# google/supersonic

Hardware: AMD Instinct MI355X
Metric: rows/sec filter->project->aggregate, 100M x 8 INT64/DOUBLE (higher is better)
Workload: dtype int64/f64; 1 GPU; Q-FPA-wide: SUM(a+b),COUNT(*),SUM(c),MIN(d),MAX(d0),SUM(d1),SUM(d2*d3) WHERE a>499 over a device-resident 100000000-row x 8-col block per GPU; rows_per_gpu=100000000, parallelism=single GPU, tile_rows=512, grid=768, lds_bytes=35568, specialized_stages=1

## Files before the change

### supersonic_amd/csrc/launch.h

```cpp
#ifndef SSGPU_LAUNCH_H_
#define SSGPU_LAUNCH_H_

#ifndef __HIPCC_RTC__
#include <hip/hip_runtime_api.h>
#include <stdint.h>
#endif
#include "vm.h"

enum SlotKind {
  SLOT_SUM_INT = 0, SLOT_SUM_DD = 1, SLOT_MIN_U64 = 2, SLOT_MAX_U64 = 3, SLOT_MIN_F64 = 4,
  SLOT_MAX_F64 = 5, SLOT_FIRST = 6, SLOT_LAST = 7, SLOT_COUNT = 8
};
enum EmitKind {
  EMIT_U64 = 0, EMIT_I64KEY = 1, EMIT_U32 = 2, EMIT_I32KEY = 3, EMIT_F64 = 4, EMIT_F32 = 5,
  EMIT_DD_F64 = 6, EMIT_DD_F32 = 7, EMIT_U8 = 8,
  EMIT_DDRES_F64 = 9,
  EMIT_CNT_U64 = 20, EMIT_CNT_U32 = 21,
  EMIT_FKEY_F64 = 100, EMIT_FKEY_F32 = 101
};
#define SSGPU_STATE_ARRAYS 8

struct EmitDesc { void* data; uint8_t* is_null; int slot; int out_kind; };

struct GroupKeyOut { void* data; uint8_t* is_null; uint32_t shift, bits, nullbit, width; };
// ... 100 lines not shown
};
hipError_t ssgpu_launch_key_domain(const PlainScatterParams& S, const unsigned int* is_signed, unsigned long long* out, int grid, hipStream_t stream);
#define SSGPU_DENSE_HEADER 64
struct DenseFoldParams {
  const void* chunks; unsigned int n_chunks, n_gaggs, any_cnt, slots;
  unsigned long long chunk_bytes;
  unsigned long long* keys; unsigned long long* acc; unsigned int* cnt;
  const unsigned int* merge_op;
  unsigned int* flags_out;
  unsigned int* clear[2]; unsigned int n_clear[2];
};
hipError_t ssgpu_launch_dense_fold(const DenseFoldParams& P, hipStream_t stream);
hipError_t ssgpu_launch_dense_headers(void* chunks, unsigned int n_chunks, unsigned long long chunk_bytes, const unsigned int* overflow4, const unsigned int* error_flag, hipStream_t stream,
                                      unsigned int forced_flags = 0);
hipError_t ssgpu_launch_hot_keys(const PlainScatterParams& S, unsigned long long n_sample, unsigned int min_count, unsigned long long* out, hipStream_t stream);
struct PscatGeom { unsigned int threads, rows, wgs_per_cu, lds, pipe; };
PscatGeom ssgpu_part_scatter_plain_geom(unsigned int n_parts, unsigned int rec_words, int threads, int rows, int wgs_per_cu);
hipError_t ssgpu_launch_part_scatter_plain(const PlainScatterParams& P, const PscatGeom& g, int grid, hipStream_t stream);
struct FoldTailColumn {
  const void* src; const unsigned char* src_nulls; void* dst; unsigned char* dst_nulls; unsigned int op, kind;
  const unsigned long long* by; const unsigned char* by_nulls;
};
hipError_t ssgpu_launch_fold_tail(const FoldTailColumn* cols_dev, unsigned int n_cols, unsigned long long n_in, unsigned long long limit, hipStream_t stream);
unsigned int ssgpu_part_scatter_plain_lds(unsigned int n_parts, unsigned int rec_words, int rows_per_thread, int threads = SSGPU_PSCAT_THREADS);
hipError_t ssgpu_part_agg_set_max_lds(int bytes);
hipError_t ssgpu_launch_group_resident(const PartAggParams& A, const PlainScatterParams& S, unsigned int lds_bytes, int grid, hipStream_t stream);

struct JoinBuildParams {
  const void* key_data[8];
  const unsigned char* key_nulls[8];
  unsigned int width[8], shift[8], bits[8];
  unsigned int n_keys;
  unsigned int capacity_mask;
  unsigned long long n_rows;
  unsigned long long* keys;
  unsigned int* rows;
  unsigned int* special;
  unsigned int* flags;
  unsigned int* counts;
  unsigned int* slot_of_row;
  unsigned int word[8];
  unsigned long long* keys_hi;
};
hipError_t ssgpu_launch_join_expand(const unsigned int* offsets, const unsigned int* run_start, const unsigned int* rows_sorted,
                                    unsigned long long n_lhs, unsigned long long n_out, unsigned int* lhs_idx, unsigned int* rhs_row, hipStream_t stream);
hipError_t ssgpu_launch_join_build(const JoinBuildParams& P, hipStream_t stream);
hipError_t ssgpu_launch_keys_ascending(const long long* keys, unsigned long long n, unsigned int* flag, hipStream_t stream);
hipError_t ssgpu_launch_fill_u32(unsigned int* p, unsigned int v, size_t n, hipStream_t stream);
struct GroupInitParams {
  unsigned long long* keys; unsigned long long n_keys;
  unsigned long long* acc; const unsigned long long* pattern; unsigned int ng; unsigned long long n_acc;
  unsigned int* cnt; unsigned long long n_cnt;
  unsigned int* z[4]; unsigned long long nz[4];
  unsigned int n_rep, pad; unsigned long long rep_stride;
};
hipError_t ssgpu_launch_group_init(const GroupInitParams& P, hipStream_t stream);

hipError_t ssgpu_launch_pipeline(const VmParams& P, int K, int grid, hipStream_t stream);
#ifndef __HIPCC_RTC__
#include <string>
void* ssgpu_rtc_specialize(int device, const VmInstr* prog, int n_instr, int K, bool math, const uint32_t* staged_width, const uint32_t* staged_lds_off,
                           int n_staged, uint32_t static_lds, std::string* why);
hipError_t ssgpu_launch_pipeline_rtc(void* handle, const VmParams& P, int grid, bool static_lds, hipStream_t stream);
void* ssgpu_rtc_specialize_part_agg(int device, const unsigned long long* desc, int n_aggs, unsigned int rec_words, unsigned int n_gaggs, bool any_cnt,
                                    unsigned int lds_bytes, std::string* why, const PlainScatterParams* source = nullptr,
                                    bool dense = false,
                                    bool prefetch = false);
hipError_t ssgpu_launch_group_resident_rtc(void* handle, const PartAggParams& A, const PlainScatterParams& S, int grid, hipStream_t stream);
hipError_t ssgpu_launch_part_agg_rtc(void* handle, const PartAggParams& P, hipStream_t stream);
void* ssgpu_rtc_specialize_pscat(int device, const PlainScatterParams& S, const PscatGeom& g, std::string* why);
hipError_t ssgpu_launch_part_scatter_plain_rtc(void* handle, const PlainScatterParams& P, const PscatGeom& g, int grid, hipStream_t stream);
void* ssgpu_rtc_function(void* handle);
void ssgpu_rtc_release(void* handle);
void ssgpu_rtc_cached_only(bool on);
void ssgpu_rtc_mode(int mode);
int ssgpu_rtc_current_mode();
bool ssgpu_rtc_pending();
void ssgpu_rtc_trim(int keep);
void ssgpu_rtc_stats(long long* modules, long long* code_bytes, long long* compilations, long long* disk_hits);
#endif
hipError_t ssgpu_pipeline_set_max_lds(int bytes);
hipError_t ssgpu_launch_finish_slots(const VmAccRec* partials, int n_slots, int n_parts, const int* slot_kind,
                                     VmAccRec* out, uint64_t* state , hipStream_t stream,
                                     const EmitDesc* descs = nullptr, int n_out = 0 );
hipError_t ssgpu_launch_slots_to_state(const VmAccRec* recs, int n_slots, const int* slot_kind, uint64_t* state,
                                       hipStream_t stream);
hipError_t ssgpu_launch_fold_state(const uint64_t* images, int n_images, uint64_t* state, int n_slots, const int* slot_kind, hipStream_t stream);
hipError_t ssgpu_launch_fold_emit(const uint64_t* images, int n_images, uint64_t* state, int n_slots, const int* slot_kind, VmAccRec* recs,
                                  const EmitDesc* descs, int n_out, hipStream_t stream);
hipError_t ssgpu_launch_state_to_slots(const uint64_t* state, int n_slots, const int* slot_kind, VmAccRec* recs,
                                       hipStream_t stream);
hipError_t ssgpu_launch_emit_scalar(const VmAccRec* recs, const EmitDesc* descs, int n_out, hipStream_t stream);
hipError_t ssgpu_launch_scan_counts(const uint32_t* in, uint32_t* out, int n, uint64_t* total, hipStream_t stream);
hipError_t ssgpu_launch_group_count(const GroupExtractParams& P, uint32_t* tile_counts, hipStream_t stream);
hipError_t ssgpu_launch_group_extract_lb(const GroupExtractParams& P, unsigned long long* status, uint64_t epoch, unsigned int* ctrl, unsigned int* error_flag, hipStream_t stream);
hipError_t ssgpu_launch_group_extract(const GroupExtractParams& P, hipStream_t stream);
hipError_t ssgpu_launch_fill_u64(uint64_t* p, uint64_t v, size_t n, hipStream_t stream);
hipError_t ssgpu_launch_fill_pattern_u64(uint64_t* p, const uint64_t* pattern, uint32_t plen, size_t n,
                                         hipStream_t stream);

hipError_t ssgpu_launch_sort_iota(uint32_t* idx, uint64_t n, hipStream_t s);
hipError_t ssgpu_launch_sort_load_keys(uint64_t* keys, const uint32_t* idx, const void* col, const uint8_t* nulls, uint32_t width,
                                       int kind, int descending, int null_pass, uint64_t n, unsigned long long* bits, hipStream_t s);
uint32_t ssgpu_sort_tiles(uint64_t n);
hipError_t ssgpu_launch_sort_hist(const uint64_t* keys, uint32_t shift, uint64_t n, uint32_t* hist, hipStream_t s);
hipError_t ssgpu_launch_sort_scatter(const uint64_t* keys_in, const uint32_t* idx_in, uint64_t* keys_out, uint32_t* idx_out,
                                     uint32_t shift, uint64_t n, const uint32_t* offsets, hipStream_t s);
hipError_t ssgpu_launch_sort_load_keys_hist(uint64_t* keys, const uint32_t* idx, const void* col, const uint8_t* nulls, uint32_t width, int kind,
                                            int descending, int null_pass, uint64_t n, unsigned long long* bits, uint32_t* hist8, uint32_t* base8, hipStream_t s,
                                            uint64_t* compact_out = nullptr);
hipError_t ssgpu_launch_sort_onesweep(const uint64_t* keys_in, const uint32_t* idx_in, uint64_t* keys_out, uint32_t* idx_out, uint32_t shift, uint64_t n,
                                      const uint32_t* digit_base, unsigned long long* status, uint32_t* ticket, uint64_t epoch, uint32_t* stuck, hipStream_t s);
hipError_t ssgpu_launch_sort_fix_ties(uint64_t* keys, uint32_t* idx, uint64_t n, uint32_t hi_shift, uint32_t* too_long, hipStream_t s);
struct SortRecField { const void* src; void* dst; unsigned int off, width; };
#define SSGPU_SORT_MAX_FIELDS 96
struct SortRecParams { void* recs; unsigned long long n; unsigned int stride, n_fields; SortRecField fields[SSGPU_SORT_MAX_FIELDS]; };
hipError_t ssgpu_launch_sort_pack(const SortRecParams& P, hipStream_t s);
hipError_t ssgpu_launch_sort_gather_rec(const SortRecParams& P, const uint32_t* idx, uint32_t idx_stride, hipStream_t s);
hipError_t ssgpu_launch_sort_fix_ties_compact(uint64_t* kc, const uint64_t* keys, uint64_t n, uint32_t* too_long, hipStream_t s);
hipError_t ssgpu_launch_sort_extract_idx(uint32_t* idx, const uint64_t* kc, uint64_t n, hipStream_t s);
struct UnpackPiece { unsigned long long src_off; void* dst; unsigned long long bytes; };
hipError_t ssgpu_launch_unpack(const char* slab, const UnpackPiece* pieces, unsigned int n_pieces, hipStream_t s);
uint64_t ssgpu_str_scan_partials(uint64_t n);
hipError_t ssgpu_launch_str_scan(uint64_t* data, uint64_t n, uint64_t* partials, hipStream_t s);
hipError_t ssgpu_launch_str_hash(const uint8_t* bytes, const uint64_t* offs, const uint8_t* nulls, uint64_t n, uint64_t* hashes, hipStream_t s);
hipError_t ssgpu_launch_str_insert(const uint8_t* bytes, const uint64_t* offs, const uint8_t* nulls, const uint64_t* hashes, uint64_t n,
                                   uint64_t* table, uint64_t cap, uint32_t* row_slot, uint32_t* error, hipStream_t s);
hipError_t ssgpu_launch_str_compact(const uint64_t* table, uint64_t cap, const uint8_t* bytes, const uint64_t* offs, uint32_t* count,
                                    uint32_t* d_slot, uint64_t* d_off, uint64_t* d_len, uint64_t* d_key, uint32_t* d_idx, hipStream_t s);
hipError_t ssgpu_launch_str_sort(uint64_t* d_key, uint32_t* d_idx, uint64_t d, uint64_t p, const uint8_t* bytes, const uint64_t* d_off,
                                 const uint64_t* d_len, hipStream_t s);
hipError_t ssgpu_launch_str_rank(const uint32_t* d_idx, const uint32_t* d_slot, const uint64_t* d_len, uint64_t d, int32_t* slot_rank,
                                 uint64_t* out_len, hipStream_t s);
hipError_t ssgpu_launch_str_codes(const uint32_t* row_slot, const uint8_t* nulls, const int32_t* slot_rank, uint64_t n, int32_t* codes, hipStream_t s);
hipError_t ssgpu_launch_str_gather(const uint8_t* bytes, const uint64_t* d_off, const uint32_t* d_idx, const uint64_t* out_off, uint64_t d,
                                   uint8_t* out, hipStream_t s);
hipError_t ssgpu_launch_str_recode(const int32_t* src, const uint8_t* nulls, const int32_t* remap, int32_t n_remap, uint64_t n, int32_t* dst,
                                   hipStream_t s);
#define STRFN_HEAP_PAD 32
hipError_t ssgpu_launch_str_fn(const uint8_t* heap, const uint64_t* offs, uint64_t n, int fn, const uint8_t* needle, uint32_t needle_len,
                               int fold, uint32_t* table, hipStream_t s);
#define STRPARSE_HARD 2
#define STRPARSE_WINDOW 64
hipError_t ssgpu_launch_str_parse(const uint8_t* heap, const uint64_t* offs, uint64_t n, int to_type, void* values, uint8_t* failed, hipStream_t s);
hipError_t ssgpu_launch_str_map_len(const uint8_t* heap, const uint64_t* offs, uint64_t n, int fn, int has_len, int64_t pos, int64_t len,
                                    uint64_t* lens, uint64_t* src, hipStream_t s);
hipError_t ssgpu_launch_str_map_write(const uint8_t* heap, const uint64_t* src, const uint64_t* dst_offs, uint64_t n, int dir, uint8_t* out, hipStream_t s);
hipError_t ssgpu_launch_str_map_compose(const int32_t* codes, uint64_t n, const int32_t* later, uint64_t n_later, uint64_t n_final, int32_t* to_final,
                                        int32_t* table, hipStream_t s);
hipError_t ssgpu_launch_str_replace_len(const uint8_t* heap, const uint64_t* offs, uint64_t n, const uint8_t* needle, uint32_t needle_len, uint32_t sub_len,
                                        uint64_t* lens, hipStream_t s);
hipError_t ssgpu_launch_str_replace_write(const uint8_t* heap, const uint64_t* offs, const uint64_t* dst_offs, uint64_t n, const uint8_t* needle, uint32_t needle_len,
                                          const uint8_t* sub, uint32_t sub_len, uint8_t* out, hipStream_t s);
hipError_t ssgpu_launch_sort_unkey(void* out, const uint64_t* keys, uint32_t width, int kind, int descending, uint64_t n, hipStream_t s);
hipError_t ssgpu_launch_sort_gather(void* out, uint8_t* out_nulls, const void* col, const uint8_t* nulls, uint32_t width,
                                    const uint32_t* idx, uint64_t n, hipStream_t s);
hipError_t ssgpu_launch_cluster_count(const void* const* data, const uint8_t* const* nulls, const uint32_t* width, uint32_t nkeys,
                                      uint64_t n, uint32_t* tile_counts, hipStream_t s);
hipError_t ssgpu_launch_cluster_flags(const void* const* data, const uint8_t* const* nulls, const uint32_t* width, uint32_t nkeys,
                                      uint64_t n, uint8_t* flag, hipStream_t s);
hipError_t ssgpu_launch_cluster_assign(const void* const* data, const uint8_t* const* nulls, const uint32_t* width, uint32_t nkeys,
                                       void* const* out_data, uint8_t* const* out_nulls, uint64_t n, const uint32_t* tile_offsets,
                                       uint32_t* seg_id, hipStream_t s);
hipError_t ssgpu_launch_gather_rowid(void* dst, const uint8_t* dst_null, const void* src, uint32_t width, int src_kind, int dst_kind, const uint64_t* rowids,
                                     uint64_t rowid_mask , int64_t row_id_base, const uint64_t* n_rows_dev, uint64_t n_rows_max, hipStream_t stream);
hipError_t ssgpu_launch_seq_sum(const void* src, const uint8_t* src_nulls, int src_kind, const uint32_t* seg_id, uint64_t n,
                                void* dst, uint8_t* dst_nulls, int dst_kind, hipStream_t s, uint64_t first = 0, uint64_t* state = nullptr, int resume = 0);
// ... 32 lines not shown
```

### supersonic_amd/csrc/pipeline_kernels.hip

```cpp
#ifndef __HIPCC_RTC__
#include <hip/hip_runtime.h>
#include <stdint.h>
#endif
#include "vm.h"
#include "launch.h"
#ifdef SSGPU_RTC_NINSTR
#include "rtc_prog.h"
#endif

typedef unsigned long long u64;
typedef long long i64;
typedef unsigned int u32;
typedef int i32;
typedef unsigned char u8;

#ifdef SSGPU_PC_PROFILE
#define PC_PROF(...) __VA_ARGS__
#else
#define PC_PROF(...)
#endif
struct LdsBase {
  __device__ __forceinline__ char* operator+(u32 off) const {
    return (char*)(__attribute__((address_space(3))) char*)off;
  }
// ... 413 lines not shown
#define KEY_APPEND_OP(OPNAME, T, UT)                                           \
  case VM_##OPNAME: { CASE_FENCE;                                              \
    const u32 shift = (u32)(I.imm & 0xFF), bits = (u32)((I.imm >> 8) & 0xFF);  \
    const u32 nullbit = (u32)((I.imm >> 16) & 0xFF);                           \
    const u64 vmask = bits >= 64 ? ~0ull : ((1ull << bits) - 1ull);            \
    _Pragma("unroll") FOR_PAIRS {                                              \
      auto kk = lds_load2<u64>(I.dst, p);                                      \
      auto vv = lds_load2<T>(I.a, p);                                          \
      u64 a0 = ((u64)(UT)vv.x) & vmask, a1 = ((u64)(UT)vv.y) & vmask;          \
      if (I.b != VM_NONE) {                                                    \
        auto z = lds_load2<u8>(I.b, p);                                        \
        if (z.x) a0 = 1ull << (nullbit - shift);                               \
        if (z.y) a1 = 1ull << (nullbit - shift);                               \
      }                                                                        \
      lds_store2<u64>(I.dst, p, kk.x | (a0 << shift), kk.y | (a1 << shift));   \
    }                                                                          \
  } break;

#define GAGG_PROLOGUE(LOADT)                                                   \
      Valid2 m = valid_pair_(p, tile_valid, I.b, VM_NONE);          \
      auto sl = lds_load2<u32>(I.c, p);                                        \
      m.x = m.x && sl.x != 0xFFFFFFFFu; m.y = m.y && sl.y != 0xFFFFFFFFu;      \
      auto vv = lds_load2<LOADT>(I.a, p);

#define GAGG_APPLY(LOADT, SL, E, ATOM)                                         \
      if ((SL) & VM_SLOT_LOCAL) {                                              \
        const u32 li = ((SL) & ~VM_SLOT_LOCAL) * P.group.local_stride + s;     \
        u64* A = reinterpret_cast<u64*>(smem + P.group.local_acc_off) + li; LOADT e = (E); ATOM; \
        if (has_cnt) atomicAdd(reinterpret_cast<u32*>(smem + P.group.local_cnt_off) + li, 1u); \
      } else {                                                                 \
        u64* A = &P.group.acc[(u64)(SL) * ng + s]; LOADT e = (E); ATOM;        \
        if (has_cnt) atomicAdd(&P.group.cnt[(u64)(SL) * ng + s], 1u);          \
      }

#define GAGG_ATOMIC(OPNAME, LOADT, ATOM)                                       \
  case VM_##OPNAME: { CASE_FENCE;                                              \
    const u32 ng = (u32)(I.imm >> 32) & 0x7FFFFFFFu, s = (u32)I.imm;           \
    const bool has_cnt = (I.imm >> 63) != 0;                                   \
    _Pragma("unroll") FOR_PAIRS {                                              \
      GAGG_PROLOGUE(LOADT)                                                     \
      if (m.x) { GAGG_APPLY(LOADT, sl.x, vv.x, ATOM) }                         \
      if (m.y) { GAGG_APPLY(LOADT, sl.y, vv.y, ATOM) }                         \
    }                                                                          \
  } break;

__device__ __noinline__ u32 lookback_rows_before(unsigned long long* status, int tile, u32 run, u64 tag, unsigned int* ctrl, unsigned int* error_flag, int lane) {
  unsigned long long* const mine = status + tile;
  if (lane == 0) __hip_atomic_store(mine, (1ull << 62) | tag | (u64)run, __ATOMIC_RELAXED, __HIP_MEMORY_SCOPE_AGENT);
  u32 excl = 0, spins = 0;
  for (int j0 = tile - 1; j0 >= 0;) {
    const int j = j0 - lane;
    u64 v = (2ull << 62) | tag;
    if (j >= 0) v = __hip_atomic_load(status + j, __ATOMIC_RELAXED, __HIP_MEMORY_SCOPE_AGENT);
    const bool ready = (v >> 62) != 0 && (v & (0x3FFFFFFFull << 32)) == tag;
    const u64 pending = __ballot(!ready), prefixes = __ballot(ready && (v >> 62) == 2);
    const u32 stop = prefixes ? (u32)__builtin_ctzll(prefixes) : 63u;
    const u64 need = stop >= 63u ? ~0ull : ((2ull << stop) - 1ull);
    if (pending & need) {
      __builtin_amdgcn_s_sleep(2);
      if (++spins > (1u << 22)) { if (lane == 0) { atomicExch(ctrl + 3, 1u); atomicExch(error_flag, 3u); } break; }
      continue;
    }
    u32 part = (u32)lane <= stop ? (u32)v : 0u;
    for (int o = 32; o > 0; o >>= 1) part += (u32)__shfl_xor((int)part, o);
    excl += part;
    if (prefixes) break;
    j0 -= 64;
  }
  if (lane == 0) __hip_atomic_store(mine, (2ull << 62) | tag | (u64)(excl + run), __ATOMIC_RELAXED, __HIP_MEMORY_SCOPE_AGENT);
  return excl;
}

__device__ __forceinline__ double vm_math1(u32 fn, double a) {
  switch (fn) {
    case VM_MATH_EXP: return exp(a);     case VM_MATH_LN: return log(a);       case VM_MATH_LOG10: return log10(a);
    case VM_MATH_LOG2: return log2(a);   case VM_MATH_SIN: return sin(a);      case VM_MATH_COS: return cos(a);
    case VM_MATH_TAN: return tan(a);     case VM_MATH_ASIN: return asin(a);    case VM_MATH_ACOS: return acos(a);
    case VM_MATH_ATAN: return atan(a);   case VM_MATH_SINH: return sinh(a);    case VM_MATH_COSH: return cosh(a);
    case VM_MATH_TANH: return tanh(a);   case VM_MATH_ASINH: return asinh(a);  case VM_MATH_ACOSH: return acosh(a);
    default: return atanh(a);
  }
}

#ifndef SSGPU_RTC_PART
template <int K, bool MATH>
__global__ __launch_bounds__(VM_WG_THREADS, VM_WAVES_PER_EU) void ssgpu_pipeline_kernel(const VmParams P) {
#ifdef SSGPU_RTC_STATIC_LDS
  __shared__ __attribute__((aligned(16))) char rtc_static_lds[SSGPU_RTC_STATIC_LDS];
  asm volatile("" ::"v"((u32)(size_t)(__attribute__((address_space(3))) char*)rtc_static_lds));
#endif
  const int t = threadIdx.x;
  const int lane = t & 63;
  const int wave = t >> 6;
  const int tile_rows = VM_TILE_UNIT * K;
  i64 vm_n_rows = P.n_rows; int vm_n_tiles = P.n_tiles;
  if (P.n_rows_dev) {
    const u64 have = *P.n_rows_dev;
    vm_n_rows = have < (u64)P.n_rows ? (i64)have : P.n_rows;
    vm_n_tiles = (int)((vm_n_rows + tile_rows - 1) / tile_rows);
  }
  const int vm_first_tile = ((P.flags & VM_FLAG_XCD_CHUNKS) && (gridDim.x & 7u) == 0u) ? (int)((blockIdx.x & 7u) * (gridDim.x >> 3) + (blockIdx.x >> 3)) : (int)blockIdx.x;
  const int n_my_tiles = vm_n_tiles > vm_first_tile ? (vm_n_tiles - vm_first_tile + (int)gridDim.x - 1) / (int)gridDim.x : 0;
  const int n_units = STAGED_COUNT(P) * K;

  for (u32 o = (u32)t * 8u; o < (u32)P.n_slots * VM_ACC_STRIDE; o += VM_COMPUTE_THREADS * 8u)
    *reinterpret_cast<u64*>(smem + P.acc_lds_off + o) = 0ull;
  typedef u64 u64xS __attribute__((ext_vector_type(VM_FAST_SLOTS)));
  typedef u32 u32xS __attribute__((ext_vector_type(VM_FAST_SLOTS)));
  u64xS F0, F1; u32xS FC;
#pragma unroll
  for (int s = 0; s < VM_FAST_SLOTS; ++s) { F0[s] = P.slot_init0[s]; F1[s] = P.slot_init1[s]; FC[s] = 0; }
  bool vm_nan_seen = false;
  for (u32 o = (u32)t * 8u; o < 2u * (u32)tile_rows; o += VM_COMPUTE_THREADS * 8u)
    *reinterpret_cast<u64*>(smem + P.const_lds_off + o) = o < (u32)tile_rows ? 0x0101010101010101ull : 0ull;

  typedef u32 u32x8 __attribute__((ext_vector_type(8)));
  typedef const __attribute__((address_space(4))) u32x8* ProgPtr;
  const ProgPtr prog0 = (ProgPtr)(P.prog);

  for (int pc = t; pc < P.n_instr; pc += VM_COMPUTE_THREADS) {
    const VmInstr J = P.prog[pc];
    const u32 w = J.imm_width;
    if (w) {
      u64 lo = J.imm;
      if (w == 4) lo = (lo & 0xFFFFFFFFull) * 0x100000001ull;
      else if (w == 1) lo = (lo & 0xFFull) * 0x0101010101010101ull;
      u64* e = reinterpret_cast<u64*>(smem + P.imm_pool_lds_off + (u32)pc * 16u);
      e[0] = lo; e[1] = lo;
    }
  }

  if (P.group.local_capacity) {
    const VmGroupTable& G = P.group;
    for (u32 e = (u32)t; e < G.local_capacity; e += VM_COMPUTE_THREADS)
      reinterpret_cast<u64*>(smem + G.local_keys_off)[e] = VM_KEY_EMPTY;
    for (u32 i = (u32)t; i < G.local_capacity * G.local_stride; i += VM_COMPUTE_THREADS) {
      reinterpret_cast<u64*>(smem + G.local_acc_off)[i] = G.acc_init[(i % G.local_stride) % G.n_gaggs];
      if (G.local_cnt_off != VM_NONE) reinterpret_cast<u32*>(smem + G.local_cnt_off)[i] = 0u;
    }
    if (t < 2) reinterpret_cast<u32*>(smem + P.scratch_lds_off + 128u)[t] = 0u;
  }
  if (P.part_n) {
    u32* h = reinterpret_cast<u32*>(smem + P.part_lds_off);
    for (u32 i = (u32)t; i < P.part_n; i += VM_COMPUTE_THREADS) h[i] = 0u;
  }
  PC_PROF(if (P.debug_pc) for (int i = t; i <= P.n_instr; i += VM_COMPUTE_THREADS) reinterpret_cast<u64*>(smem + P.debug_pc_lds_off)[i] = 0ull;)
  __syncthreads();

  u32x4 pf[VM_PF_UNITS];
#pragma unroll
  for (int u = 0; u < VM_PF_UNITS; ++u) pf[u] = u32x4{0u, 0u, 0u, 0u};
  const int n_pf = n_units < VM_PF_UNITS ? n_units : VM_PF_UNITS;
  {
    const i64 tb = (i64)vm_first_tile * tile_rows;
    if (n_my_tiles > 0 && tb + tile_rows <= vm_n_rows) {
#pragma unroll
      for (int u = 0; u < VM_PF_UNITS; ++u)
        if (u < n_pf) load_unit<K>(P, u, tb, t, pf[u]);
    }
  }

  u64 dbg_wait = 0;
  const u64 dbg_t0 = P.debug ? __builtin_amdgcn_s_memtime() : 0;
  const ProgPtr prog = prog0;
  for (int it = 0; it < n_my_tiles; ++it) {
    const int tile = vm_first_tile + it * (int)gridDim.x;
    const i64 tile_base = (i64)tile * tile_rows;
    const u32 tile_valid = (u32)((vm_n_rows - tile_base) < (i64)tile_rows ? (vm_n_rows - tile_base) : (i64)tile_rows);
    const u64 tw0 = (P.debug || P.debug_pc) ? __builtin_amdgcn_s_memtime() : 0;
    __builtin_amdgcn_s_setprio(VM_STAGE_PRIO);
    if (tile_valid == (u32)tile_rows) {
      int tc = t;
      asm volatile("" : "+v"(tc));
#pragma unroll
      for (int u = 0; u < VM_PF_UNITS; ++u)
        if (u < n_pf) commit_unit<K>(P, u, pf[u], tc);
      if (P.debug) dbg_wait += __builtin_amdgcn_s_memtime() - tw0;
      if (n_units > VM_PF_UNITS) stage_units_direct<K>(P, VM_PF_UNITS, n_units, tile_base, tile_valid, t);
    } else {
      stage_units_direct<K>(P, 0, n_units, tile_base, tile_valid, t);
    }
    {
      const i64 tb = tile_base + (i64)gridDim.x * tile_rows;
      if (it + 1 < n_my_tiles && tb + tile_rows <= vm_n_rows) {
        int tl = t;
        asm volatile("" : "+v"(tl));
#pragma unroll
        for (int u = 0; u < VM_PF_UNITS; ++u)
          if (u < n_pf) load_unit<K>(P, u, tb, tl, pf[u]);
      }
    }

    __builtin_amdgcn_s_setprio(0);
#ifdef SSGPU_RTC_NINSTR
#define VM_PC_LOOP _Pragma("unroll") for (int pc = 0; pc < SSGPU_RTC_NINSTR; ++pc)
#define VM_FETCH_NEXT(pc) u32x8{kRtcProg[pc][0], kRtcProg[pc][1], kRtcProg[pc][2], kRtcProg[pc][3], kRtcProg[pc][4], kRtcProg[pc][5], kRtcProg[pc][6], kRtcProg[pc][7]}
    (void)prog;
    u32x8 raw_next = VM_FETCH_NEXT(0);
#else
#define VM_PC_LOOP for (int pc = 0; pc < P.n_instr; ++pc)
#define VM_FETCH_NEXT(pc) prog[pc]
    u32x8 raw_next = prog[0];
#endif
    PC_PROF(u64 dbg_pc_last = 0;
    if (P.debug_pc) { dbg_pc_last = __builtin_amdgcn_s_memtime(); if (t == 0) reinterpret_cast<u64*>(smem + P.debug_pc_lds_off)[P.n_instr] += dbg_pc_last - tw0; })
#ifdef SSGPU_RTC_NINSTR
#include "rtc_steps.h"
#else
    VM_PC_LOOP {
#include "vm_body.inc"
    }
#endif
    PC_PROF(if (P.debug_pc && P.n_instr > 0 && t == 0) reinterpret_cast<u64*>(smem + P.debug_pc_lds_off)[P.n_instr - 1] += __builtin_amdgcn_s_memtime() - dbg_pc_last;)
  }

  if (vm_nan_seen && P.error_flag) atomicOr(P.error_flag, SSGPU_FLAG_NAN_IN_MINMAX);
  if (P.part_n && P.tile_counts) {
    __syncthreads();
    const u32* h = reinterpret_cast<const u32*>(smem + P.part_lds_off);
    for (u32 i = (u32)t; i < P.part_n; i += VM_COMPUTE_THREADS) P.tile_counts[(u64)i * gridDim.x + blockIdx.x] = h[i] < P.part_seg_cap ? h[i] : P.part_seg_cap;
  }
  if (P.group.local_capacity) {
    const VmGroupTable& G = P.group;
    __syncthreads();
    const u32 ng = G.n_gaggs;
    u32 occupied = 0;
    for (u32 e = (u32)t; e < G.local_capacity; e += VM_COMPUTE_THREADS) {
      const u64 key = reinterpret_cast<const u64*>(smem + G.local_keys_off)[e];
      if (key == VM_KEY_EMPTY) continue;
      ++occupied;
      const u32 gs = group_insert(G, key);
      if (gs == 0xFFFFFFFFu) continue;
      for (u32 s = 0; s < ng; ++s) {
        const u64 v = reinterpret_cast<const u64*>(smem + G.local_acc_off)[e * G.local_stride + s];
        u64* A = &G.acc[(u64)gs * ng + s];
        const u32 op = G.merge_op[s];
        if (op == VM_MERGE_ADD_U64) { if (v) atomicAdd(A, v); }
        else if (op == VM_MERGE_MIN_U64) atomicMin(A, v);
        else if (op == VM_MERGE_MAX_U64) atomicMax(A, v);
        else if (op == VM_MERGE_ADD_F64_HI) dd_atomic_add(reinterpret_cast<double*>(A), u2d(v));
        else unsafeAtomicAdd(reinterpret_cast<double*>(A), u2d(v));
        if (G.local_cnt_off != VM_NONE) {
          const u32 c = reinterpret_cast<const u32*>(smem + G.local_cnt_off)[e * G.local_stride + s];
          if (c) atomicAdd(&G.cnt[(u64)gs * ng + s], c);
        }
      }
    }
    u32* st = reinterpret_cast<u32*>(smem + P.scratch_lds_off + 128u);
    if (occupied) atomicAdd(&st[1], occupied);
    __syncthreads();
    if (t == 0) { if (st[0]) atomicAdd(&G.stats[0], st[0]); atomicMax(&G.stats[1], st[1]); }
  }

  PC_PROF(if (P.debug_pc && t == 0) for (int i = 0; i <= P.n_instr; ++i) atomicAdd(&P.debug_pc[i], reinterpret_cast<const u64*>(smem + P.debug_pc_lds_off)[i]);)
  if (P.debug && t == 0) {
    P.debug[blockIdx.x * 4 + 0] = __builtin_amdgcn_s_memtime() - dbg_t0;
    P.debug[blockIdx.x * 4 + 1] = dbg_wait;
    P.debug[blockIdx.x * 4 + 2] = (u64)n_my_tiles;
  }
#pragma unroll
  for (int s = 0; s < VM_FAST_SLOTS; ++s) {
    if (s < P.n_slots) {
      const int kind = P.slot_kind[s];
      const u64 cnt = wave_reduce_u64((u64)FC[s], [](u64 x, u64 y) { return x + y; });
      u64 v0 = 0, v1 = 0;
      switch (kind) {
        case SLOT_COUNT: v0 = cnt; break;
        case SLOT_SUM_INT: v0 = wave_reduce_u64(F0[s], [](u64 x, u64 y) { return x + y; }); break;
        case SLOT_MIN_U64: v0 = wave_reduce_u64(F0[s], [](u64 x, u64 y) { return x < y ? x : y; }); break;
        case SLOT_MAX_U64: v0 = wave_reduce_u64(F0[s], [](u64 x, u64 y) { return x > y ? x : y; }); break;
        case SLOT_MIN_F64: v0 = wave_reduce_u64(F0[s], [](u64 x, u64 y) { return u2d(y) < u2d(x) ? y : x; }); break;
        case SLOT_MAX_F64: v0 = wave_reduce_u64(F0[s], [](u64 x, u64 y) { return u2d(x) < u2d(y) ? y : x; }); break;
        case SLOT_SUM_DD: {
          DD d; d.hi = u2d(F0[s]); d.lo = u2d(F1[s]);
          d = wave_reduce_dd(d); v0 = d2u(d.hi); v1 = d2u(d.lo);
        } break;
        case SLOT_FIRST: case SLOT_LAST: {
          const bool first = kind == SLOT_FIRST;
          const u64 trow = first ? wave_reduce_u64(F1[s], [](u64 x, u64 y) { return x < y ? x : y; })
                                 : wave_reduce_u64(FC[s] ? F1[s] : 0ull, [](u64 x, u64 y) { return x > y ? x : y; });
          const u64 owner = __ballot(FC[s] != 0 && F1[s] == trow);
          const int src = owner ? __ffsll((long long)owner) - 1 : 0;
          v0 = readlane64(F0[s], src); v1 = trow;
        } break;
        default: break;
      }
      if (lane == 0) { VmAccRec* A = acc_rec(P, (u32)s, wave); A->v0 = v0; A->v1 = v1; A->cnt = cnt; A->pad = 0; }
    }
  }

  __syncthreads();
  for (int s = t; s < P.n_slots; s += VM_COMPUTE_THREADS)
    for (int w = 0; w < VM_WAVES; ++w)
      P.wg_partials[((size_t)blockIdx.x * P.n_slots + s) * VM_WAVES + w] = *acc_rec(P, (u32)s, w);
}
#endif

#ifndef __HIPCC_RTC__

__device__ __forceinline__ void combine_rec(int kind, VmAccRec& acc, const VmAccRec& r) {
  if (r.cnt == 0) return;
  switch (kind) {
    case SLOT_COUNT:
    case SLOT_SUM_INT: acc.v0 += r.v0; break;
    case SLOT_SUM_DD: {
      DD a; a.hi = u2d(acc.v0); a.lo = u2d(acc.v1);
      DD b; b.hi = u2d(r.v0); b.lo = u2d(r.v1);
      a = dd_add(a, b); acc.v0 = d2u(a.hi); acc.v1 = d2u(a.lo);
    } break;
    case SLOT_MIN_U64: acc.v0 = acc.cnt ? (r.v0 < acc.v0 ? r.v0 : acc.v0) : r.v0; break;
    case SLOT_MAX_U64: acc.v0 = acc.cnt ? (r.v0 > acc.v0 ? r.v0 : acc.v0) : r.v0; break;
    case SLOT_MIN_F64: acc.v0 = acc.cnt ? (u2d(r.v0) < u2d(acc.v0) ? r.v0 : acc.v0) : r.v0; break;
    case SLOT_MAX_F64: acc.v0 = acc.cnt ? (u2d(acc.v0) < u2d(r.v0) ? r.v0 : acc.v0) : r.v0; break;
    case SLOT_FIRST: if (!acc.cnt || r.v1 < acc.v1) { acc.v0 = r.v0; acc.v1 = r.v1; } break;
    case SLOT_LAST: if (!acc.cnt || r.v1 >= acc.v1) { acc.v0 = r.v0; acc.v1 = r.v1; } break;
  }
  acc.cnt += r.cnt;
}

__device__ __forceinline__ void slot_to_state(const VmAccRec r, int kind, int s, int n_slots, u64* __restrict__ state) {
  u64* sum_i = state; u64* cnt = state + n_slots; u64* hi = state + 2 * n_slots; u64* lo = state + 3 * n_slots;
  u64* mn = state + 4 * n_slots; u64* mx = state + 5 * n_slots;
  u64* mnf = state + 6 * n_slots; u64* mxf = state + 7 * n_slots;
  const bool fl = kind == SLOT_FIRST || kind == SLOT_LAST;
  sum_i[s] = (kind == SLOT_SUM_INT || kind == SLOT_COUNT || fl) ? r.v0 : 0;
  cnt[s] = r.cnt;
  hi[s] = kind == SLOT_SUM_DD ? r.v0 : d2u(0.0);
  lo[s] = kind == SLOT_SUM_DD ? r.v1 : d2u(0.0);
  mn[s] = (kind == SLOT_MIN_U64 && r.cnt) ? (r.v0 ^ 0x8000000000000000ull) : (kind == SLOT_FIRST && r.cnt) ? (r.v1 ^ 0x8000000000000000ull) : 0x7FFFFFFFFFFFFFFFull;
  mx[s] = (kind == SLOT_MAX_U64 && r.cnt) ? (r.v0 ^ 0x8000000000000000ull) : (kind == SLOT_LAST && r.cnt) ? (r.v1 ^ 0x8000000000000000ull) : 0x8000000000000000ull;
  mnf[s] = (kind == SLOT_MIN_F64 && r.cnt) ? r.v0 : d2u(__builtin_inf());
  mxf[s] = (kind == SLOT_MAX_F64 && r.cnt) ? r.v0 : d2u(-__builtin_inf());
}
__device__ __forceinline__ VmAccRec state_to_slot(const u64* __restrict__ state, int kind, int s, int n_slots) {
  VmAccRec r; r.v0 = 0; r.v1 = 0; r.pad = 0;
  r.cnt = state[n_slots + s];
  switch (kind) {
    case SLOT_COUNT: case SLOT_SUM_INT: r.v0 = state[s]; break;
    case SLOT_SUM_DD: {
      DD a; a.hi = u2d(state[2 * n_slots + s]); a.lo = 0.0;
      a = dd_add_d(a, u2d(state[3 * n_slots + s]));
      r.v0 = d2u(a.hi); r.v1 = d2u(a.lo);
    } break;
    case SLOT_MIN_U64: r.v0 = state[4 * n_slots + s] ^ 0x8000000000000000ull; break;
    case SLOT_MAX_U64: r.v0 = state[5 * n_slots + s] ^ 0x8000000000000000ull; break;
    case SLOT_MIN_F64: r.v0 = state[6 * n_slots + s]; break;
    case SLOT_MAX_F64: r.v0 = state[7 * n_slots + s]; break;
    case SLOT_FIRST: r.v0 = state[s]; r.v1 = state[4 * n_slots + s] ^ 0x8000000000000000ull; break;
    case SLOT_LAST: r.v0 = state[s]; r.v1 = state[5 * n_slots + s] ^ 0x8000000000000000ull; break;
    default: break;
  }
  return r;
}

__device__ __forceinline__ void emit_scalar_one(const EmitDesc d, const VmAccRec r);
__global__ __launch_bounds__(256) void ssgpu_finish_slots_kernel(const VmAccRec* __restrict__ partials, int n_slots,
                                                                 int n_parts, const int* __restrict__ slot_kind,
                                                                 VmAccRec* __restrict__ out, u64* __restrict__ state,
                                                                 const EmitDesc* __restrict__ descs, int n_out) {
  __shared__ VmAccRec tree[256];
  const int s = blockIdx.x, t = threadIdx.x;
  const int kind = slot_kind[s];
  VmAccRec acc; acc.v0 = 0; acc.v1 = 0; acc.cnt = 0; acc.pad = 0;
  if (kind == SLOT_SUM_DD) { acc.v0 = d2u(-0.0); acc.v1 = d2u(0.0); }
  for (int i = t; i < n_parts; i += 256) {
    const VmAccRec r = partials[((size_t)(i / VM_WAVES) * n_slots + s) * VM_WAVES + (i % VM_WAVES)];
    combine_rec(kind, acc, r);
  }
  tree[t] = acc;
  __syncthreads();
  for (int stride = 128; stride > 0; stride >>= 1) {
    if (t < stride) { VmAccRec a = tree[t]; combine_rec(kind, a, tree[t + stride]); tree[t] = a; }
    __syncthreads();
  }
  if (t == 0) { out[s] = tree[0]; if (state) slot_to_state(tree[0], kind, s, n_slots, state); }
  if (descs)
    for (int i = t; i < n_out; i += 256) { const EmitDesc d = descs[i]; if (d.slot == s) emit_scalar_one(d, tree[0]); }
}

__global__ void ssgpu_slots_to_state_kernel(const VmAccRec* __restrict__ recs, int n_slots,
                                            const int* __restrict__ slot_kind, u64* __restrict__ state) {
  int s = blockIdx.x * blockDim.x + threadIdx.x;
  if (s >= n_slots) return;
  slot_to_state(recs[s], slot_kind[s], s, n_slots, state);
}
__global__ void ssgpu_state_to_slots_kernel(const u64* __restrict__ state, int n_slots,
                                            const int* __restrict__ slot_kind, VmAccRec* __restrict__ recs) {
  int s = blockIdx.x * blockDim.x + threadIdx.x;
  if (s >= n_slots) return;
  recs[s] = state_to_slot(state, slot_kind[s], s, n_slots);
}


__device__ __forceinline__ void emit_value(void* dst, size_t idx, int out_kind, u64 v0, u64 v1) {
  switch (out_kind) {
    case EMIT_U64: reinterpret_cast<u64*>(dst)[idx] = v0; break;
    case EMIT_I64KEY: reinterpret_cast<i64*>(dst)[idx] = unkey_i64(v0); break;
    case EMIT_U32: reinterpret_cast<u32*>(dst)[idx] = (u32)v0; break;
    case EMIT_I32KEY: reinterpret_cast<i32*>(dst)[idx] = (i32)unkey_i64(v0); break;
    case EMIT_F64: reinterpret_cast<double*>(dst)[idx] = u2d(v0); break;
    case EMIT_F32: reinterpret_cast<float*>(dst)[idx] = (float)u2d(v0); break;
    case EMIT_DD_F64: { double hi = u2d(v0), lo = u2d(v1);
      reinterpret_cast<double*>(dst)[idx] = (lo == 0.0) ? hi : hi + lo; } break;
    case EMIT_DDRES_F64: { const double hi = u2d(v0), lo = u2d(v1), sm = hi + lo, bp = sm - hi;
      reinterpret_cast<double*>(dst)[idx] = (lo == 0.0) ? 0.0 : (hi - (sm - bp)) + (lo - bp); } break;
    case EMIT_DD_F32: { double hi = u2d(v0), lo = u2d(v1);
      reinterpret_cast<float*>(dst)[idx] = (float)((lo == 0.0) ? hi : hi + lo); } break;
    case EMIT_U8: reinterpret_cast<u8*>(dst)[idx] = (u8)(v0 != 0); break;
    default: break;
  }
}


__device__ __forceinline__ void emit_scalar_one(const EmitDesc d, const VmAccRec r) {
  if (d.out_kind == EMIT_CNT_U64 || d.out_kind == EMIT_CNT_U32)
    emit_value(d.data, 0, d.out_kind == EMIT_CNT_U64 ? EMIT_U64 : EMIT_U32, r.cnt, 0);
  else
    emit_value(d.data, 0, d.out_kind, r.v0, r.v1);
  if (d.is_null) d.is_null[0] = r.cnt == 0;
}
__global__ void ssgpu_emit_scalar_kernel(const VmAccRec* __restrict__ recs, const EmitDesc* __restrict__ descs,
                                         int n_out) {
  int i = blockIdx.x * blockDim.x + threadIdx.x;
  if (i >= n_out) return;
  const EmitDesc d = descs[i];
  emit_scalar_one(d, recs[d.slot]);
}

__global__ __launch_bounds__(1024) void ssgpu_scan_counts_kernel(const u32* __restrict__ in, u32* __restrict__ out,
                                                                  int n, u64* __restrict__ total) {
  __shared__ u64 wave_sums[16];
  __shared__ u64 carry_s;
  const int t = threadIdx.x, lane = t & 63, wave = t >> 6;
  if (t == 0) carry_s = 0;
  __syncthreads();
  for (int base = 0; base < n; base += 1024 * 8) {
    u32 v[8]; u64 sum = 0;
    int i0 = base + t * 8;
#pragma unroll
    for (int j = 0; j < 8; ++j) { v[j] = (i0 + j < n) ? in[i0 + j] : 0u; sum += v[j]; }
    u64 inc = sum;
#pragma unroll
    for (int d = 1; d < 64; d <<= 1) { u64 o = __shfl_up(inc, d); if (lane >= d) inc += o; }
    if (lane == 63) wave_sums[wave] = inc;
    __syncthreads();
    u64 wpre = 0;
    for (int w = 0; w < wave; ++w) wpre += wave_sums[w];
    u64 run = carry_s + wpre + (inc - sum);
#pragma unroll
    for (int j = 0; j < 8; ++j) { if (i0 + j < n) out[i0 + j] = (u32)run; run += v[j]; }
    __syncthreads();
    if (t == 1023) carry_s = run;
    __syncthreads();
  }
  if (t == 0) *total = carry_s;
}

__device__ __forceinline__ bool group_slot_occupied(const GroupExtractParams& P, u32 slot) {
  if (slot > P.capacity + P.extra_slots) return false;
  return P.keys[slot] != VM_KEY_EMPTY;
}

__global__ __launch_bounds__(256) void ssgpu_group_count_kernel(const GroupExtractParams P, u32* __restrict__ tile_counts) {
  __shared__ u32 wsum[4];
  const int t = threadIdx.x, lane = t & 63, wave = t >> 6;
  u32 s0 = blockIdx.x * 512u + t * 2u;
  bool o0 = group_slot_occupied(P, s0);
  bool o1 = group_slot_occupied(P, s0 + 1);
  u32 c = (u32)__popcll(__ballot(o0)) + (u32)__popcll(__ballot(o1));
  if (lane == 0) wsum[wave] = c;
  __syncthreads();
  if (t == 0) tile_counts[blockIdx.x] = wsum[0] + wsum[1] + wsum[2] + wsum[3];
}

__device__ __forceinline__ void group_extract_slot(const GroupExtractParams& P, u32 slot, u32 row);
__global__ __launch_bounds__(256) void ssgpu_group_extract_lb_kernel(const GroupExtractParams P, unsigned long long* __restrict__ status, u64 tag,
                                                                     unsigned int* __restrict__ ctrl, unsigned int* __restrict__ error_flag) {
  __shared__ u32 wsum[4];
  __shared__ u32 s_tile, s_base;
  const int t = threadIdx.x, lane = t & 63, wave = t >> 6;
  if (t == 0) s_tile = atomicAdd(ctrl + 2, 1u);
  __syncthreads();
  const u32 tile = s_tile;
  const u32 s0 = tile * 512u + (u32)t * 2u;
  const bool o0 = group_slot_occupied(P, s0), o1 = group_slot_occupied(P, s0 + 1);
  const u64 b0 = __ballot(o0), b1 = __ballot(o1);
  if (lane == 0) wsum[wave] = (u32)__popcll(b0) + (u32)__popcll(b1);
  __syncthreads();
  if (wave == 0) {
    const u32 run = wsum[0] + wsum[1] + wsum[2] + wsum[3];
    const u32 excl = lookback_rows_before(status, (int)tile, run, tag, ctrl, error_flag, lane);
    if (lane == 0) {
      s_base = excl;
      if (tile == gridDim.x - 1u) *reinterpret_cast<u64*>(ctrl) = (u64)excl + run;
    }
  }
  __syncthreads();
  u32 base = s_base;
  for (int w = 0; w < wave; ++w) base += wsum[w];
  const u64 lt = (1ull << lane) - 1ull;
  const u32 r0 = base + (u32)__popcll(b0 & lt) + (u32)__popcll(b1 & lt);
  if (o0) group_extract_slot(P, s0, r0);
  if (o1) group_extract_slot(P, s0 + 1, r0 + (o0 ? 1u : 0u));
// ... 785 lines not shown
__global__ __launch_bounds__(256) void ssgpu_gather_rowid_kernel(void* __restrict__ dst, const u8* __restrict__ dst_null, const void* __restrict__ src,
                                                                 u32 width, int src_kind, int dst_kind, const u64* __restrict__ rowids, u64 rowid_mask, i64 row_id_base,
                                                                 const u64* __restrict__ n_rows_dev, u64 n_rows_max) {
  const u64 i = (u64)blockIdx.x * 256 + threadIdx.x;
  const u64 n = n_rows_dev ? *n_rows_dev : n_rows_max;
  if (i >= n || i >= n_rows_max) return;
  const bool isnull = dst_null && dst_null[i];
  const u64 r = isnull ? 0ull : (u64)((i64)(rowids[i] & rowid_mask) - row_id_base);
  if (src_kind == dst_kind) {
    if (width == 8) reinterpret_cast<u64*>(dst)[i] = isnull ? 0ull : reinterpret_cast<const u64*>(src)[r];
    else if (width == 4) reinterpret_cast<u32*>(dst)[i] = isnull ? 0u : reinterpret_cast<const u32*>(src)[r];
    else reinterpret_cast<u8*>(dst)[i] = isnull ? (u8)0 : reinterpret_cast<const u8*>(src)[r];
    return;
  }
  i64 vi = 0; u64 vu = 0; double vf = 0.0; int fam = 0;
  if (!isnull) switch (src_kind) {
    case 0: vi = reinterpret_cast<const i32*>(src)[r]; fam = 0; break;
    case 1: vu = reinterpret_cast<const u32*>(src)[r]; fam = 1; break;
    case 2: vi = reinterpret_cast<const i64*>(src)[r]; fam = 0; break;
    case 3: vu = reinterpret_cast<const u64*>(src)[r]; fam = 1; break;
    case 4: vf = (double)reinterpret_cast<const float*>(src)[r]; fam = 2; break;
    case 5: vf = reinterpret_cast<const double*>(src)[r]; fam = 2; break;
    default: vu = reinterpret_cast<const u8*>(src)[r]; fam = 1; break;
  }
  if (dst_kind == 4 || dst_kind == 5) {
    const double d = fam == 2 ? vf : (fam == 1 ? (double)vu : (double)vi);
    if (dst_kind == 5) reinterpret_cast<double*>(dst)[i] = d;
    else reinterpret_cast<float*>(dst)[i] = fam == 2 ? (float)vf : (fam == 1 ? (float)vu : (float)vi);
    return;
  }
  u64 bits;
  if (fam == 2) {
    const double tr = trunc(vf);
    bits = (tr >= -9223372036854775808.0 && tr < 9223372036854775808.0) ? (u64)(i64)tr : 0x8000000000000000ull;
  } else bits = fam == 1 ? vu : (u64)vi;
  if (dst_kind == 2 || dst_kind == 3) reinterpret_cast<u64*>(dst)[i] = bits;
  else if (dst_kind == 0 || dst_kind == 1) reinterpret_cast<u32*>(dst)[i] = (u32)bits;
  else reinterpret_cast<u8*>(dst)[i] = (u8)bits;
}
hipError_t ssgpu_launch_gather_rowid(void* dst, const uint8_t* dst_null, const void* src, uint32_t width, int src_kind, int dst_kind, const uint64_t* rowids, uint64_t rowid_mask,
                                     int64_t row_id_base, const uint64_t* n_rows_dev, uint64_t n_rows_max, hipStream_t stream) {
  if (n_rows_max) hipLaunchKernelGGL(ssgpu_gather_rowid_kernel, dim3((unsigned)((n_rows_max + 255) / 256)), dim3(256), 0, stream,
                                     dst, dst_null, src, width, src_kind, dst_kind, (const u64*)rowids, (u64)rowid_mask, (i64)row_id_base, (const u64*)n_rows_dev, (u64)n_rows_max);
  return hipGetLastError();
}
hipError_t ssgpu_launch_fill_u32(unsigned int* p, unsigned int v, size_t n, hipStream_t stream) {
  if (n) hipLaunchKernelGGL(ssgpu_fill_u32_kernel, dim3((unsigned)std::min<size_t>((n + 255) / 256, 4096)), dim3(256), 0, stream, p, v, n);
  return hipGetLastError();
}
hipError_t ssgpu_launch_part_agg(const PartAggParams& P, unsigned int lds_bytes, hipStream_t stream) {
  if (P.rec_words <= 8) hipLaunchKernelGGL(ssgpu_part_agg_kernel<8>, dim3(P.n_parts), dim3(SSGPU_PART_THREADS), lds_bytes, stream, P);
  else if (P.rec_words <= 16) hipLaunchKernelGGL(ssgpu_part_agg_kernel<16>, dim3(P.n_parts), dim3(SSGPU_PART_THREADS), lds_bytes, stream, P);
  else if (P.rec_words <= SSGPU_PART_MAX_WORDS) hipLaunchKernelGGL(ssgpu_part_agg_kernel<SSGPU_PART_MAX_WORDS>, dim3(P.n_parts), dim3(SSGPU_PART_THREADS), lds_bytes, stream, P);
  else return hipErrorInvalidValue;
  return hipGetLastError();
}
hipError_t ssgpu_launch_group_resident(const PartAggParams& P, const PlainScatterParams& S, unsigned int lds_bytes, int grid, hipStream_t stream) {
  if (P.rec_words <= 8) hipLaunchKernelGGL(ssgpu_group_resident_kernel<8>, dim3(grid), dim3(SSGPU_PART_THREADS), lds_bytes, stream, P, S);
  else hipLaunchKernelGGL(ssgpu_group_resident_kernel<16>, dim3(grid), dim3(SSGPU_PART_THREADS), lds_bytes, stream, P, S);
  return hipGetLastError();
}
hipError_t ssgpu_part_agg_set_max_lds(int bytes) {
  hipError_t e = hipFuncSetAttribute(reinterpret_cast<const void*>(ssgpu_part_agg_kernel<8>), hipFuncAttributeMaxDynamicSharedMemorySize, bytes);
  if (e != hipSuccess) return e;
  e = hipFuncSetAttribute(reinterpret_cast<const void*>(ssgpu_group_resident_kernel<8>), hipFuncAttributeMaxDynamicSharedMemorySize, bytes);
  if (e != hipSuccess) return e;
  e = hipFuncSetAttribute(reinterpret_cast<const void*>(ssgpu_group_resident_kernel<16>), hipFuncAttributeMaxDynamicSharedMemorySize, bytes);
  if (e != hipSuccess) return e;
  e = hipFuncSetAttribute(reinterpret_cast<const void*>(ssgpu_part_agg_kernel<SSGPU_PART_MAX_WORDS>), hipFuncAttributeMaxDynamicSharedMemorySize, bytes);
  if (e != hipSuccess) return e;
  return hipFuncSetAttribute(reinterpret_cast<const void*>(ssgpu_part_agg_kernel<16>), hipFuncAttributeMaxDynamicSharedMemorySize, bytes);
}
hipError_t ssgpu_pipeline_set_max_lds(int bytes) {
  hipError_t e;
  e = hipFuncSetAttribute(reinterpret_cast<const void*>(ssgpu_pipeline_kernel<1, false>), hipFuncAttributeMaxDynamicSharedMemorySize, bytes); if (e != hipSuccess) return e;
  e = hipFuncSetAttribute(reinterpret_cast<const void*>(ssgpu_pipeline_kernel<2, false>), hipFuncAttributeMaxDynamicSharedMemorySize, bytes); if (e != hipSuccess) return e;
  e = hipFuncSetAttribute(reinterpret_cast<const void*>(ssgpu_pipeline_kernel<4, false>), hipFuncAttributeMaxDynamicSharedMemorySize, bytes); if (e != hipSuccess) return e;
  e = hipFuncSetAttribute(reinterpret_cast<const void*>(ssgpu_pipeline_kernel<1, true>), hipFuncAttributeMaxDynamicSharedMemorySize, bytes); if (e != hipSuccess) return e;
  e = hipFuncSetAttribute(reinterpret_cast<const void*>(ssgpu_pipeline_kernel<2, true>), hipFuncAttributeMaxDynamicSharedMemorySize, bytes); if (e != hipSuccess) return e;
  e = hipFuncSetAttribute(reinterpret_cast<const void*>(ssgpu_pipeline_kernel<4, true>), hipFuncAttributeMaxDynamicSharedMemorySize, bytes);
  return e;
}
hipError_t ssgpu_launch_finish_slots(const VmAccRec* partials, int n_slots, int n_parts, const int* slot_kind,
                                     VmAccRec* out, uint64_t* state, hipStream_t stream, const EmitDesc* descs, int n_out) {
  hipLaunchKernelGGL(ssgpu_finish_slots_kernel, dim3(n_slots), dim3(256), 0, stream, partials, n_slots, n_parts, slot_kind, out, (u64*)state, descs, n_out);
  return hipGetLastError();
}
hipError_t ssgpu_launch_slots_to_state(const VmAccRec* recs, int n_slots, const int* slot_kind, uint64_t* state, hipStream_t stream) {
  int blocks = (n_slots + 63) / 64;
  hipLaunchKernelGGL(ssgpu_slots_to_state_kernel, dim3(blocks), dim3(64), 0, stream, recs, n_slots, slot_kind, (u64*)state);
  return hipGetLastError();
}
__device__ __forceinline__ void fold_state_slot(const u64* __restrict__ images, int n_images, u64* __restrict__ state, int n_slots, int kind, int s);
__global__ __launch_bounds__(64) void ssgpu_fold_state_kernel(const u64* __restrict__ images, int n_images, u64* __restrict__ state,
                                                              int n_slots, const int* __restrict__ slot_kind) {
  const int s = blockIdx.x * 64 + threadIdx.x;
  if (s >= n_slots) return;
  fold_state_slot(images, n_images, state, n_slots, slot_kind[s], s);
}
__device__ __forceinline__ void fold_state_slot(const u64* __restrict__ images, int n_images, u64* __restrict__ state, int n_slots, int kind, int s) {
  const size_t total = (size_t)SSGPU_STATE_ARRAYS * n_slots;
  u64 a[SSGPU_STATE_ARRAYS];
  for (int k = 0; k < SSGPU_STATE_ARRAYS; ++k) a[k] = images[(size_t)k * n_slots + s];
  for (int r = 1; r < n_images; ++r) {
    u64 v[SSGPU_STATE_ARRAYS];
    for (int k = 0; k < SSGPU_STATE_ARRAYS; ++k) v[k] = images[(size_t)r * total + (size_t)k * n_slots + s];
    if (kind == SLOT_FIRST) { if ((i64)v[4] < (i64)a[4]) a[0] = v[0]; }
    else if (kind == SLOT_LAST) { if ((i64)v[5] > (i64)a[5]) a[0] = v[0]; }
    else a[0] += v[0];
    a[1] += v[1];
    a[2] = d2u(u2d(a[2]) + u2d(v[2]));
    a[3] = d2u(u2d(a[3]) + u2d(v[3]));
    a[4] = (i64)v[4] < (i64)a[4] ? v[4] : a[4];
    a[5] = (i64)v[5] > (i64)a[5] ? v[5] : a[5];
    a[6] = u2d(v[6]) < u2d(a[6]) ? v[6] : a[6];
    a[7] = u2d(v[7]) > u2d(a[7]) ? v[7] : a[7];
  }
  for (int k = 0; k < SSGPU_STATE_ARRAYS; ++k) state[(size_t)k * n_slots + s] = a[k];
}
__global__ __launch_bounds__(256) void ssgpu_fold_emit_kernel(const u64* __restrict__ images, int n_images, u64* __restrict__ state, int n_slots,
                                                              const int* __restrict__ slot_kind, VmAccRec* __restrict__ recs,
                                                              const EmitDesc* __restrict__ descs, int n_out) {
  for (int s = threadIdx.x; s < n_slots; s += 256) {
    fold_state_slot(images, n_images, state, n_slots, slot_kind[s], s);
    recs[s] = state_to_slot(state, slot_kind[s], s, n_slots);
  }
  __threadfence_block();
  __syncthreads();
  for (int i = threadIdx.x; i < n_out; i += 256) { const EmitDesc d = descs[i]; emit_scalar_one(d, recs[d.slot]); }
}
hipError_t ssgpu_launch_fold_emit(const uint64_t* images, int n_images, uint64_t* state, int n_slots, const int* slot_kind, VmAccRec* recs,
                                  const EmitDesc* descs, int n_out, hipStream_t stream) {
  hipLaunchKernelGGL(ssgpu_fold_emit_kernel, dim3(1), dim3(256), 0, stream, (const u64*)images, n_images, (u64*)state, n_slots, slot_kind, recs, descs, n_out);
  return hipGetLastError();
}
hipError_t ssgpu_launch_fold_state(const uint64_t* images, int n_images, uint64_t* state, int n_slots, const int* slot_kind, hipStream_t stream) {
  if (n_slots > 0) hipLaunchKernelGGL(ssgpu_fold_state_kernel, dim3((n_slots + 63) / 64), dim3(64), 0, stream, (const u64*)images, n_images, (u64*)state, n_slots, slot_kind);
  return hipGetLastError();
}
hipError_t ssgpu_launch_state_to_slots(const uint64_t* state, int n_slots, const int* slot_kind, VmAccRec* recs, hipStream_t stream) {
  int blocks = (n_slots + 63) / 64;
  hipLaunchKernelGGL(ssgpu_state_to_slots_kernel, dim3(blocks), dim3(64), 0, stream, (const u64*)state, n_slots, slot_kind, recs);
  return hipGetLastError();
}
hipError_t ssgpu_launch_emit_scalar(const VmAccRec* recs, const EmitDesc* descs, int n_out, hipStream_t stream) {
  int blocks = (n_out + 63) / 64;
  hipLaunchKernelGGL(ssgpu_emit_scalar_kernel, dim3(blocks), dim3(64), 0, stream, recs, descs, n_out);
  return hipGetLastError();
}
__global__ __launch_bounds__(1024) void ssgpu_scan_chunk_totals_kernel(const u32* __restrict__ in, int n, u32* __restrict__ totals) {
  __shared__ u64 wave_sums[16];
  const int t = threadIdx.x, lane = t & 63, wave = t >> 6;
  const int i0 = blockIdx.x * 8192 + t * 8;
  u64 sum = 0;
#pragma unroll
  for (int j = 0; j < 8; ++j) sum += (i0 + j < n) ? in[i0 + j] : 0u;
#pragma unroll
  for (int d = 32; d > 0; d >>= 1) sum += __shfl_xor(sum, d);
  if (lane == 0) wave_sums[wave] = sum;
  __syncthreads();
  if (t == 0) { u64 s = 0; for (int w = 0; w < 16; ++w) s += wave_sums[w]; totals[blockIdx.x] = (u32)s; }
}
__global__ __launch_bounds__(1024) void ssgpu_scan_chunks_kernel(const u32* __restrict__ in, u32* __restrict__ out, int n,
                                                                  const u32* __restrict__ chunk_base) {
  __shared__ u64 wave_sums[16];
  const int t = threadIdx.x, lane = t & 63, wave = t >> 6;
  const int i0 = blockIdx.x * 8192 + t * 8;
  u32 v[8]; u64 sum = 0;
// ... 64 lines not shown
```

### supersonic_amd/csrc/runtime.cpp

```cpp
#include <hip/hip_runtime_api.h>

#include <atomic>
#include <chrono>
#include <map>
#include <set>
#include <mutex>
#include <stdio.h>
#include <stdlib.h>
#include <string.h>
#include <algorithm>
#include <array>
#include <cmath>
#include <string>
#include <unistd.h>
#include <thread>
#include <unordered_set>
#include <vector>
#include <deque>
#include <functional>

#include "runtime_internal.h"

using namespace ssgpu;

// ... 13 lines not shown
    for (auto it = blocks.begin(); it != blocks.end();)
      if (dev < 0 || it->second.second == dev) { out.emplace_back(it->second.first, it->first); bytes -= it->first; it = blocks.erase(it); } else ++it;
  }
  size_t freed = 0;
  for (auto& b : out) { (void)hipFree(b.first); g_dev_bytes.fetch_sub((long long)b.second); freed += b.second; }
  return freed;
}
static std::atomic<int> g_device_contexts{0};
thread_local bool tls_park_released = false;

struct OutCol { DevBuf data, nulls; bool nullable = false; uint32_t width = 8; };

struct StageExec {
  DevBuf prog_main, prog_count;
  struct RtcSlot {
    void* h = nullptr; bool tried = false; uint32_t static_lds = 0, tag = 0;
    int missed_mode = -1;
    bool stronger_mode_now() const { if (h || missed_mode < 0) return false; const int m = ssgpu_rtc_current_mode(); return missed_mode == 1 && m != 1; }
    bool pending = false; std::chrono::steady_clock::time_point next_poll{};
    void drop() { if (h) ssgpu_rtc_release(h); h = nullptr; tried = false; static_lds = 0; tag = 0; pending = false; missed_mode = -1; }
    bool ask_again() {
      if (!pending) return false;
      const auto now = std::chrono::steady_clock::now();
      if (now < next_poll) return false;
      next_poll = now + std::chrono::milliseconds(20);
      return true;
    }
    void asked() { pending = !h && ssgpu_rtc_pending(); missed_mode = h ? -1 : ssgpu_rtc_current_mode(); if (pending) next_poll = std::chrono::steady_clock::now() + std::chrono::milliseconds(20); }
  };
  RtcSlot rtc_main;
  std::vector<VmInstr> host_prog_main;
  std::string rtc_why;
  ProgramLayout lay{};
  ProgramLayout lay_count{};
  int n_instr_main = 0, n_instr_count = 0;
  int grid = 0;
  DevBuf wg_partials, slot_recs, slot_kind, emit_descs, state;
  DevBuf tile_counts, tile_offsets, total;
  DevBuf xstatus; uint64_t x_epoch = 0;
  DevBuf gkeys, gacc, gcnt, goverflow, gpattern, gmergeop;
  int group_wgs = 3;
  bool group_local = true;
  int group_sub = 1;
  bool group_partitioned = false;
  uint32_t part_n = 256;
  bool part_n_chosen = false;
  bool part_slab_failed = false;
  bool scouted = false;
  int64_t scout_full_rows = 0;
  bool part_slab = false;
  double part_groups_est = 0;
  uint32_t part_seg_growth = 1;
  bool part_failed = false;
  DevBuf prog_pscatter, part_hist, part_recs;
  ProgramLayout lay_pscatter{};
  int n_instr_pscatter = 0;
  RtcSlot rtc_pscatter; std::vector<VmInstr> host_prog_pscatter;
  RtcSlot rtc_plain;
  RtcSlot rtc_part;
  RtcSlot rtc_resident;
  RtcSlot rtc_hot;
  uint32_t hot_n = 0; uint64_t hot_keys[SSGPU_HOT_MAX] = {0};
  int64_t hot_sampled_run = -1;
  DevBuf hot_out;
  struct DenseState {
    bool on = false, failed = false, checked = false, fixed = false, resident = false;
    uint32_t n_keys = 0, n_chunks = 1;
    uint64_t lo[8] = {0}, hi[8] = {0};
    uint32_t span[8] = {0}, stride[8] = {0};
    uint64_t slots = 0;
    uint32_t np = 0, cap = 0;
    uint64_t chunk_bytes = 0;
    int64_t widened = 0;
  } dense;
  DevBuf dense_dom, dense_flags;
  void* dense_table = nullptr;
  std::vector<DevBuf> rowid_tmp;
  std::vector<DevBuf> jkeys, jkeys_hi, jrows, jmisc;
  std::vector<DevBuf> jcounts, jstarts, jslot_of_row, jrows_sorted;
  DevBuf jx_offsets, jx_lhs_idx, jx_rhs_row;
  std::vector<VmJoin> vm_joins;
  uint32_t capacity = 0;
  DevBuf error_flag;
  DevBuf debug, debug_pc, total2;
  DevBuf skeys_a, skeys_b, skeys_c, sidx_a, sidx_b, shist, soffs, seg_id, sstatus, sticket, srecs, dflag;
  DevBuf rank_first, rank_of_seg, rank_row, rank_own;
  DevBuf seg_counts, seg_offsets, seg_total;
  DevBuf route_scratch;
  uint64_t sort_epoch = 0;
  bool emit_ready = false;
  bool emitted_with_finish = false;
  bool pattern_ready = false;
  DevBuf out_arena;
  std::vector<OutCol> out;
  int64_t out_rows = -1;
  const void* out_rows_dev = nullptr;
  int64_t out_capacity = 0;
  int last_group_shape = 0;
  int last_reruns = 0;
  int last_sort_passes = 0, last_sort_mode = 0;
  bool last_plain_scatter = false;
  PinnedBuf fb_host;
  int fb_pending = 0;
  hipEvent_t fb_event = nullptr;
  int steady = 0;
  uint32_t steady_bypass = 0;
};

struct ssgpu_result {
  ssgpu_plan* plan = nullptr;
  std::vector<PinnedBuf> host_data, host_nulls;
  std::vector<bool> fetched;
  std::vector<ssgpu_dict*> concat_dicts;
  ~ssgpu_result() { for (ssgpu_dict* d : concat_dicts) if (d) ssgpu_dict_destroy(d); }
};

struct ssgpu_plan {
  ssgpu_ctx* ctx = nullptr;
  MemQuota quota;
  int64_t expr_row_capacity = INT64_MAX;
  PlanDesc desc;
  std::vector<Stage> stages;
  std::vector<StageExec> exec;
  Schema result_schema;
  std::vector<std::string> attr_names;
  std::vector<ssgpu_column> aux_cols;
  int64_t aux_rows = -1;
  std::string describe, describe_full;
  std::atomic<int> interrupted{0};
  int64_t n_runs = 0;
  bool specialize = false;
  bool cached_only = false;
  bool best_effort = false; int64_t be_cut = -1, be_capacity = 0, be_window = 0, be_base = 0, be_window_fail = 0;
  uint32_t group_capacity_hint = 0;
  bool lazy_feedback = false;
  bool background = false;
  int64_t background_min_rows = 0;
  hipEvent_t ev_begin = nullptr, ev_end = nullptr, ev_dom0 = nullptr, ev_dom1 = nullptr;
  static const int kEventRing = 256;
  hipEvent_t ring0[kEventRing] = {nullptr}, ring1[kEventRing] = {nullptr};
  uint64_t profiled_runs = 0;
  bool events_valid = false;
  ssgpu_counters counters{};
  std::vector<VmInstr> host_prog_scratch;
  bool partial_pending = false;
  int64_t last_rows = 0;
  bool deferred = false;
  bool nan_seen = false;
  const ssgpu_dict* dict = nullptr;
  uint64_t dict_gen = 0;
  DictTables dict_tables;
  std::vector<ssgpu_column> last_cols; int64_t last_base = 0; bool last_partial = false;
  std::vector<DevBuf> host_stage_data[2], host_stage_nulls[2];
  DevBuf host_states;
  struct HostStream {
    bool open = false; int rc = SSGPU_OK;
    int64_t chunk_rows = 0, fill = 0, pushed = 0, chunks = 0; int cur = 0;
    int kind = 1;
    std::vector<PinnedBuf> pin_data[2], pin_nulls[2];
    hipEvent_t uploaded[2] = {nullptr, nullptr}, consumed[2] = {nullptr, nullptr};
    bool in_flight[2] = {false, false};
    void drop_events() {
      for (int b = 0; b < 2; ++b) {
        if (uploaded[b]) (void)hipEventDestroy(uploaded[b]);
        if (consumed[b]) (void)hipEventDestroy(consumed[b]);
        uploaded[b] = consumed[b] = nullptr; in_flight[b] = false;
// ... 51 lines not shown
  if (device_id >= 0) {
    int n = 0;
    hipError_t e = hipGetDeviceCount(&n);
    if (e != hipSuccess || device_id >= n) { delete c; return SSGPU_ERROR_NO_DEVICE; }
    if (hipSetDevice(device_id) != hipSuccess) { delete c; return SSGPU_ERROR_NO_DEVICE; }
    hipDeviceProp_t prop;
    if (hipGetDeviceProperties(&prop, device_id) != hipSuccess) { delete c; return SSGPU_ERROR_NO_DEVICE; }
    c->cu_count = prop.multiProcessorCount;
    if (hipStreamCreateWithFlags(&c->stream, hipStreamNonBlocking) != hipSuccess ||
        hipStreamCreateWithFlags(&c->copy_stream, hipStreamNonBlocking) != hipSuccess) { delete c; return SSGPU_ERROR_HIP; }
    c->own_stream = true;
    g_device_contexts.fetch_add(1);
    (void)ssgpu_pipeline_set_max_lds(160 * 1024);
    (void)ssgpu_part_agg_set_max_lds(160 * 1024);
  }
  if (const char* e = getenv("SSGPU_SPECIALIZE")) c->specialize = atoi(e);
  if (const char* e = getenv("SSGPU_GROUP_DENSE")) c->group_dense = atoi(e);
  *out = c;
  return SSGPU_OK;
}

static void ctx_release(ssgpu_ctx* c) {
  if (c->refs.fetch_sub(1) != 1) return;
  if (c->device >= 0) {
    if (c->own_stream && c->stream) (void)hipStreamDestroy(c->stream);
    if (c->copy_stream) (void)hipStreamDestroy(c->copy_stream);
    if (c->copy_ev) { (void)hipEventDestroy(c->copy_ev); c->copy_ev = nullptr; }
    if (g_device_contexts.fetch_sub(1) == 1) (void)g_pool.trim(-1);
  }
  delete c;
}
int64_t ssgpu_pool_trim(int32_t device) { return (int64_t)g_pool.trim(device); }
void ssgpu_ctx_destroy(ssgpu_ctx* c) { if (c) ctx_release(c); }

int ssgpu_ctx_has_device(const ssgpu_ctx* c) { return c && c->device >= 0 ? 1 : 0; }
const char* ssgpu_last_error(const ssgpu_ctx* c) { return c ? c->err.c_str() : "null context"; }
void* ssgpu_ctx_stream(ssgpu_ctx* c) { return c ? (void*)c->stream : nullptr; }
void* ssgpu_ctx_copy_stream(ssgpu_ctx* c) { return c ? (void*)c->copy_stream : nullptr; }

int ssgpu_ctx_set_stream(ssgpu_ctx* c, void* s) {
  if (!c || c->device < 0) return SSGPU_ERROR_NO_DEVICE;
  if (c->own_stream && c->stream) (void)hipStreamDestroy(c->stream);
  c->stream = (hipStream_t)s; c->own_stream = false;
  return SSGPU_OK;
}

int ssgpu_ctx_synchronize(ssgpu_ctx* c) {
  if (!c || c->device < 0) return SSGPU_ERROR_NO_DEVICE;
  HIP_TRY(c, hipStreamSynchronize(c->stream));
  HIP_TRY(c, hipStreamSynchronize(c->copy_stream));
  return SSGPU_OK;
}

int ssgpu_ctx_set_option(ssgpu_ctx* c, const char* key, int64_t value) {
  if (!c || !key) return SSGPU_ERROR_INVALID_ARGUMENT_VALUE;
  std::string k(key);
  if (k == "tile_rows") {
    if (value != 0 && (value % VM_TILE_UNIT != 0 || value > 4 * VM_TILE_UNIT)) { c->err = "tile_rows must be 0 or 1, 2, 4 times the workgroup's row-pair count"; return SSGPU_ERROR_INVALID_ARGUMENT_VALUE; }
    c->opt.tile_rows = (int)value;
  } else if (k == "lds_target_bytes") c->opt.lds_target_bytes = (int)value;
  else if (k == "grid_limit") c->grid_limit = value;
  else if (k == "wgs_per_cu") c->wgs_per_cu = value > 0 ? value : 3;
  else if (k == "tile_map") c->tile_map = value;
  else if (k == "out_arena") c->out_arena = value;
  else if (k == "group_local") c->group_local = value;
  else if (k == "group_partition") c->group_partition = value;
  else if (k == "part_n") c->part_n = value;
  else if (k == "part_wgs_per_cu") c->part_wgs_per_cu = value;
  else if (k == "part_lds_target") c->part_lds_target = value;
  else if (k == "part_agg_lds") c->part_agg_lds = value;
  else if (k == "group_slab") c->group_slab = value;
  else if (k == "group_resident") c->group_resident = value;
  else if (k == "group_dense") c->group_dense = value;
  else if (k == "dense_parts") c->dense_parts = value;
  else if (k == "dense_min_rows") c->dense_min_rows = value;
  else if (k == "group_scout") c->group_scout = value;
  else if (k == "group_scout_rows") c->group_scout_rows = value;
  else if (k == "part_plain") c->part_plain = value;
  else if (k == "pscat_threads") c->pscat_threads = value;
  else if (k == "pscat_rows") c->pscat_rows = value;
  else if (k == "pscat_wgs") c->pscat_wgs = value;
  else if (k == "pscat_pipe") c->pscat_pipe = value;
  else if (k == "fuse_emit") c->fuse_emit = value;
  else if (k == "part_prefetch") c->part_prefetch = value;
  else if (k == "lazy_feedback") c->lazy_feedback = value;
  else if (k == "async_handoff") c->async_handoff = value;
  else if (k == "sort_records") c->sort_records = value;
  else if (k == "sort_hybrid") c->sort_hybrid = value;
  else if (k == "sort_hi_digits") c->sort_hi_digits = value;
  else if (k == "sort_compact") c->sort_compact = value;
  else if (k == "group_capacity") {
    int64_t cap = 1; while (cap < value) cap <<= 1;
    c->group_capacity = cap;
  } else if (k == "profile") c->profile = value;
  else if (k == "profile_total") c->profile_total = value;
  else if (k == "debug_timing") c->debug_timing = value;
  else if (k == "specialize") c->specialize = value;
  else if (k == "specialize_min_rows") c->specialize_min_rows = value < 0 ? 0 : value;
  else { c->err = "unknown option " + k; return SSGPU_ERROR_INVALID_ARGUMENT_VALUE; }
  return SSGPU_OK;
}

int ssgpu_host_alloc(ssgpu_ctx* c, size_t bytes, void** out) {
  if (!c || c->device < 0) return SSGPU_ERROR_NO_DEVICE;
  HIP_TRY(c, hipHostMalloc(out, std::max<size_t>(bytes, 1), hipHostMallocDefault));
  return SSGPU_OK;
}
void ssgpu_host_free(ssgpu_ctx* c, void* p) { (void)c; if (p) (void)hipHostFree(p); }

int ssgpu_block_create(ssgpu_ctx* c, const ssgpu_attr* schema, int32_t n, int64_t cap, ssgpu_block** out) {
  if (!c || c->device < 0) return SSGPU_ERROR_NO_DEVICE;
  ssgpu_block* b = new ssgpu_block;
  b->ctx = c; b->capacity = cap; b->rows = 0;
  b->data.resize(n); b->nulls.resize(n);
  size_t total = 0;
  for (int i = 0; i < n; ++i) {
    Attr a; a.name = schema[i].name ? schema[i].name : ""; a.dtype = schema[i].dtype; a.nullable = schema[i].nullable != 0;
    int w = dtype_width(a.dtype);
    if (w == 0) { delete b; c->err = "variable-length columns are outside the device hot path"; return SSGPU_ERROR_NOT_IMPLEMENTED; }
    b->schema.push_back(a);
    total += (size_t)cap * w + (a.nullable ? (size_t)cap : 0);
  }
  if (total >= kBlockArenaMin) {
    auto pitch = [](size_t bytes) { return ((bytes + (2u << 20) - 1) / (2u << 20)) * (2u << 20) + kBlockColumnSkew; };
    size_t need = 0;
    for (int i = 0; i < n; ++i) need += pitch((size_t)cap * dtype_width(b->schema[i].dtype)) + (b->schema[i].nullable ? pitch((size_t)cap) : 0);
    if (b->arena.ensure(need) != hipSuccess) { delete b; c->err = "device allocation failed"; return SSGPU_ERROR_MEMORY_EXCEEDED; }
    size_t off = 0;
    for (int i = 0; i < n; ++i) { const size_t bytes = (size_t)cap * dtype_width(b->schema[i].dtype); b->data[i].set_view(b->arena.as<char>() + off, bytes); off += pitch(bytes); }
    for (int i = 0; i < n; ++i) if (b->schema[i].nullable) { b->nulls[i].set_view(b->arena.as<char>() + off, (size_t)cap); off += pitch((size_t)cap); }
  } else {
    for (int i = 0; i < n; ++i) {
      if (b->data[i].ensure((size_t)cap * dtype_width(b->schema[i].dtype)) != hipSuccess) { delete b; c->err = "device allocation failed"; return SSGPU_ERROR_MEMORY_EXCEEDED; }
      if (b->schema[i].nullable && b->nulls[i].ensure((size_t)cap) != hipSuccess) { delete b; c->err = "device allocation failed"; return SSGPU_ERROR_MEMORY_EXCEEDED; }
    }
  }
  c->refs.fetch_add(1);
  g_live_blocks.fetch_add(1);
  *out = b;
  return SSGPU_OK;
}
void ssgpu_block_destroy(ssgpu_block* b) { if (!b) return; ssgpu_ctx* c = b->ctx; ssgpu_dict_destroy(b->dict); delete b; g_live_blocks.fetch_sub(1); if (c) ctx_release(c); }

static const int64_t kFileChunkRows = 8192;

static bool read_slab(FILE* f, char* dst, size_t bytes) {
  const long pos = ftell(f);
  const int fd = fileno(f);
  const int kReaders = bytes >= (8u << 20) ? 4 : 1;
  const size_t part = (bytes + kReaders - 1) / kReaders;
  std::atomic<bool> ok{true};
  auto read_part = [&](int i) {
    size_t lo = (size_t)i * part, hi = std::min(bytes, lo + part);
    while (lo < hi) {
      const ssize_t got = pread(fd, dst + lo, hi - lo, (off_t)(pos + (long)lo));
      if (got <= 0) { ok = false; return; }
      lo += (size_t)got;
    }
  };
  std::vector<std::thread> readers;
  for (int i = 1; i < kReaders; ++i) readers.emplace_back(read_part, i);
  read_part(0);
  for (auto& t : readers) t.join();
  return ok && fseek(f, pos + (long)bytes, SEEK_SET) == 0;
}

// ... 367 lines not shown
  out->dtype = p->result_schema[i].dtype;
  out->nullable = p->result_schema[i].nullable ? 1 : 0;
  return SSGPU_OK;
}
const char* ssgpu_plan_describe(ssgpu_plan* p) {
  if (!p) return "";
  std::string lines;
  for_each_dict_table(p, true, [&](const DictTableSpec& spec) { lines += p->dict_tables.describe(spec, p->dict); });
  if (lines.empty()) return p->describe.c_str();
  p->describe_full = p->describe + lines;
  return p->describe_full.c_str();
}

int ssgpu_plan_program(const ssgpu_plan* cp, int32_t stage, const void** instrs, int32_t* n, int32_t* bytes) {
  ssgpu_plan* p = const_cast<ssgpu_plan*>(cp);
  if (!p || stage < 0 || stage >= (int)p->stages.size()) return SSGPU_ERROR_INVALID_ARGUMENT_VALUE;
  ProgramLayout L = layout_program(p->stages[stage].main, p->ctx->opt);
  finalize_program(p->stages[stage].main, L, &p->host_prog_scratch);
  *instrs = p->host_prog_scratch.data(); *n = (int32_t)p->host_prog_scratch.size(); *bytes = (int32_t)sizeof(VmInstr);
  return SSGPU_OK;
}

void ssgpu_interrupt(ssgpu_plan* p) { if (p) p->interrupted.store(1, std::memory_order_relaxed); }

}

namespace {

struct InCols { std::vector<ssgpu_column> cols; int64_t rows = 0;
                const unsigned long long* rows_dev = nullptr; };

int upload_program(ssgpu_ctx* c, const Program& prog, const ProgramLayout& L, DevBuf* dev, int* n_instr, std::vector<VmInstr>* scratch) {
  finalize_program(prog, L, scratch);
  *n_instr = (int)prog.code.size();
  HIP_TRY(c, dev->ensure(std::max<size_t>(1, scratch->size()) * sizeof(VmInstr)));
  if (!scratch->empty())
    HIP_TRY(c, hipMemcpyAsync(dev->p, scratch->data(), scratch->size() * sizeof(VmInstr), hipMemcpyHostToDevice, c->stream));
  HIP_TRY(c, hipStreamSynchronize(c->stream));
  return SSGPU_OK;
}

static void staged_table(const Program& prog, const ProgramLayout& L, std::vector<uint32_t>* width, std::vector<uint32_t>* off) {
  width->clear(); off->clear();
  for (auto& sgd : prog.staged) { width->push_back(prog.regs[sgd.reg].width); off->push_back(prog.regs[sgd.reg].row_off * (uint32_t)(VM_TILE_UNIT * L.K)); }
}
void* rtc_for(ssgpu_plan* p, StageExec& ex, StageExec::RtcSlot& slot, const Program& prog, const ProgramLayout& L, const std::vector<VmInstr>& host_prog,
              int n_instr, uint32_t lds_bytes, const char* what) {
  if (!p->specialize) return nullptr;
  ssgpu_ctx* c = p->ctx;
  const uint32_t need_static = lds_bytes > 64u * 1024u ? ((lds_bytes + 15u) & ~15u) : 0u;
  if (slot.tried && slot.static_lds == need_static && !slot.ask_again() && !slot.stronger_mode_now()) return slot.h;
  if (slot.h) { (void)hipStreamSynchronize(c->stream); slot.drop(); }
  const bool was_pending = slot.pending;
  slot.tried = true; slot.static_lds = need_static;
  std::vector<uint32_t> sw, so; staged_table(prog, L, &sw, &so);
  std::string why;
  slot.h = ssgpu_rtc_specialize(c->device, host_prog.data(), n_instr, L.K, prog.uses_math, sw.data(), so.data(), (int)sw.size(), need_static, &why);
  slot.asked();
  if (!slot.h && ex.rtc_why.empty()) ex.rtc_why = std::string(what) + why;
  if (slot.h && was_pending) ex.rtc_why.clear();
  return slot.h;
}

int prepare_stage(ssgpu_plan* p, size_t si) {
  ssgpu_ctx* c = p->ctx;
  Stage& st = p->stages[si];
  StageExec& ex = p->exec[si];
  if (st.main.empty()) return SSGPU_OK;
  ProgramLayout L = layout_program(st.main, c->opt);
  if (ex.prog_main.p && L.K == ex.lay.K) return SSGPU_OK;
  ex.lay = L;
  int rc = upload_program(c, st.main, L, &ex.prog_main, &ex.n_instr_main, &p->host_prog_scratch);
  if (rc != SSGPU_OK) return rc;
  ex.host_prog_main = p->host_prog_scratch;
  if (ex.rtc_main.h) (void)hipStreamSynchronize(c->stream);
  ex.rtc_main.drop(); ex.rtc_why.clear();
  if (!st.count_pass.empty()) {
    LowerOptions o = c->opt; o.tile_rows = VM_TILE_UNIT * 4;
    ex.lay_count = layout_program(st.count_pass, o);
    if (ex.lay_count.K < L.K) { o.tile_rows = VM_TILE_UNIT * L.K; ex.lay_count = layout_program(st.count_pass, o); }
    rc = upload_program(c, st.count_pass, ex.lay_count, &ex.prog_count, &ex.n_instr_count, &p->host_prog_scratch);
    if (rc != SSGPU_OK) return rc;
  }
  HIP_TRY(c, ex.error_flag.ensure(sizeof(uint32_t)));
  return SSGPU_OK;
}

int sort_rows_by_u32(ssgpu_plan* p, StageExec& ex, const uint32_t* keys32, uint64_t n, uint32_t** sorted) {
  ssgpu_ctx* c = p->ctx;
  const uint32_t nt = ssgpu_sort_tiles(n);
  HIP_TRY(c, ex.skeys_a.ensure(std::max<uint64_t>(n, 1) * 8)); HIP_TRY(c, ex.skeys_b.ensure(std::max<uint64_t>(n, 1) * 8));
  HIP_TRY(c, ex.sidx_a.ensure(std::max<uint64_t>(n, 1) * 4)); HIP_TRY(c, ex.sidx_b.ensure(std::max<uint64_t>(n, 1) * 4));
  HIP_TRY(c, ex.shist.ensure((size_t)std::max<uint32_t>(nt, 1) * 256 * 4)); HIP_TRY(c, ex.soffs.ensure((size_t)std::max<uint32_t>(nt, 1) * 256 * 4));
  HIP_TRY(c, ex.total.ensure(8)); HIP_TRY(c, ex.total2.ensure(16));
  uint64_t* ka = ex.skeys_a.as<uint64_t>(); uint64_t* kb = ex.skeys_b.as<uint64_t>();
  uint32_t* ia = ex.sidx_a.as<uint32_t>(); uint32_t* ib = ex.sidx_b.as<uint32_t>();
  HIP_TRY(c, ssgpu_launch_sort_iota(ia, n, c->stream));
  if (n > 0) {
    const unsigned long long init[2] = {0ull, ~0ull};
    HIP_TRY(c, hipMemcpyAsync(ex.total2.p, init, 16, hipMemcpyHostToDevice, c->stream));
    HIP_TRY(c, ssgpu_launch_sort_load_keys(ka, ia, keys32, nullptr, 4, 0, 0, 0, n, ex.total2.as<unsigned long long>(), c->stream));
    unsigned long long bits[2];
    HIP_TRY(c, hipMemcpyAsync(bits, ex.total2.p, 16, hipMemcpyDeviceToHost, c->stream));
    HIP_TRY(c, hipStreamSynchronize(c->stream));
    const uint64_t varying = bits[0] ^ bits[1];
    for (uint32_t pass = 0; pass < 4; ++pass) {
      if (!((varying >> (pass * 8)) & 0xFFull)) continue;
      HIP_TRY(c, ssgpu_launch_sort_hist(ka, pass * 8, n, ex.shist.as<uint32_t>(), c->stream));
      HIP_TRY(c, ssgpu_launch_scan_counts(ex.shist.as<uint32_t>(), ex.soffs.as<uint32_t>(), (int)(nt * 256), ex.total.as<uint64_t>(), c->stream));
      HIP_TRY(c, ssgpu_launch_sort_scatter(ka, ia, kb, ib, pass * 8, n, ex.soffs.as<uint32_t>(), c->stream));
      std::swap(ka, kb); std::swap(ia, ib);
      p->counters.n_launches += 3;
    }
  }
  *sorted = ia;
  return SSGPU_OK;
}

int build_joins(ssgpu_plan* p, Stage& st, StageExec& ex) {
  ssgpu_ctx* c = p->ctx;
  if (st.joins.empty()) return SSGPU_OK;
  if (p->aux_rows < 0) { c->err = "this plan joins against an auxiliary input: call ssgpu_plan_set_aux_input first"; return SSGPU_ERROR_INVALID_ARGUMENT_VALUE; }
  const size_t nj = st.joins.size();
  ex.jkeys.resize(nj); ex.jkeys_hi.resize(nj); ex.jrows.resize(nj); ex.jmisc.resize(nj); ex.vm_joins.resize(nj);
  for (size_t j = 0; j < nj; ++j) {
    const JoinSpec& js = st.joins[j];
    if (js.form != JoinSpec::HASH) {
      VmJoin& J = ex.vm_joins[j];
      memset(&J, 0, sizeof(J));
      J.capacity_mask = (uint32_t)p->aux_rows;
      if (js.form == JoinSpec::SEARCH) {
        const long long* keys = static_cast<const long long*>(p->aux_cols[js.rhs_key_cols[0]].data);
        if (p->aux_rows > 0 && !keys) { c->err = "ForeignFilter: the filter's key column has no data"; return SSGPU_ERROR_INVALID_ARGUMENT_VALUE; }
        J.keys = reinterpret_cast<const unsigned long long*>(keys);
        if (p->aux_rows > 1) {
          HIP_TRY(c, ex.jmisc[j].ensure(16));
          HIP_TRY(c, hipMemsetAsync(ex.jmisc[j].p, 0, 16, c->stream));
          HIP_TRY(c, ssgpu_launch_keys_ascending(keys, (unsigned long long)p->aux_rows, ex.jmisc[j].as<unsigned int>(), c->stream));
          uint32_t unordered = 0;
          HIP_TRY(c, hipMemcpyAsync(&unordered, ex.jmisc[j].p, 4, hipMemcpyDeviceToHost, c->stream));
          HIP_TRY(c, hipStreamSynchronize(c->stream));
          p->counters.n_launches += 1;
          if (unordered) { c->err = "ForeignFilter: the filter keys must be unique and ascending (a key is not greater than the one before it)"; return SSGPU_ERROR_INVALID_ARGUMENT_VALUE; }
        }
      }
      continue;
    }
    uint64_t cap = 16; while (cap < (uint64_t)std::max<int64_t>(p->aux_rows, 1) * 2) cap <<= 1;
    if (cap > (1ull << 31)) { c->err = "hash join rhs table too large"; return SSGPU_ERROR_MEMORY_EXCEEDED; }
    HIP_TRY(c, ex.jmisc[j].ensure(16));
    if (js.wide) {
      HIP_TRY(c, ex.jkeys[j].ensure(cap * 8)); HIP_TRY(c, ex.jkeys_hi[j].ensure(cap * 8)); HIP_TRY(c, ex.jrows[j].ensure(cap * 4));
      HIP_TRY(c, ssgpu_launch_fill_u32(ex.jrows[j].as<unsigned int>(), VM_NONE, cap, c->stream));
    } else {
      HIP_TRY(c, ex.jkeys[j].ensure(cap * 16));
      HIP_TRY(c, ssgpu_launch_fill_u64(ex.jkeys[j].as<uint64_t>(), VM_KEY_EMPTY, cap * 2, c->stream));
    }
    const uint32_t misc_init[4] = {VM_NONE, 0u, 0u, 0u};
    HIP_TRY(c, hipMemcpyAsync(ex.jmisc[j].p, misc_init, 16, hipMemcpyHostToDevice, c->stream));
    JoinBuildParams B; memset(&B, 0, sizeof(B));
    B.n_keys = (unsigned)js.rhs_key_cols.size();
    for (size_t k = 0; k < js.rhs_key_cols.size(); ++k) {
      const ssgpu_column& col = p->aux_cols[js.rhs_key_cols[k]];
      B.key_data[k] = col.data; B.key_nulls[k] = p->desc.aux_schema[js.rhs_key_cols[k]].nullable ? col.is_null : nullptr;
      B.width[k] = js.fields[k].width; B.shift[k] = js.fields[k].shift; B.bits[k] = js.fields[k].bits; B.word[k] = js.fields[k].word;
    }
    B.capacity_mask = (uint32_t)(cap - 1); B.n_rows = (unsigned long long)p->aux_rows;
// ... 125 lines not shown
  P->scratch_lds_off = L.scratch_off;
  P->imm_pool_lds_off = L.imm_pool_off;
  P->const_lds_off = L.imm_pool_off + 16u * (uint32_t)prog.code.size();
  P->lds_bytes = L.lds_bytes;
  for (size_t i = 0; i < prog.staged.size(); ++i) {
    const StagedInput& s = prog.staged[i];
    P->staged[i].src = s.is_null_mask ? (const void*)in.cols[s.col].is_null : in.cols[s.col].data;
    P->staged[i].lds_off = prog.regs[s.reg].row_off * (uint32_t)P->tile_rows;
    P->staged[i].width = prog.regs[s.reg].width;
  }
}

int ensure_out_cols(ssgpu_ctx* c, const Stage& st, StageExec& ex, int64_t rows) {
  ex.out.resize(st.out_schema.size());
  size_t total = 0;
  for (size_t i = 0; i < st.out_schema.size(); ++i) {
    OutCol& oc = ex.out[i];
    oc.width = (uint32_t)dtype_width(st.out_schema[i].dtype);
    oc.nullable = st.out_schema[i].nullable;
    total += (size_t)std::max<int64_t>(rows, 1) * (oc.width + (oc.nullable ? 1u : 0u));
  }
  if (c->out_arena && total >= kBlockArenaMin && st.out_schema.size() > 1) {
    auto pitch = [](size_t bytes) { return ((bytes + (2u << 20) - 1) / (2u << 20)) * (2u << 20) + kBlockColumnSkew; };
    bool fits = ex.out_arena.p != nullptr;
    for (size_t i = 0; i < ex.out.size() && fits; ++i)
      fits = ex.out[i].data.view && ex.out[i].data.cap >= (size_t)std::max<int64_t>(rows, 1) * ex.out[i].width + 16 &&
             (!ex.out[i].nullable || (ex.out[i].nulls.view && ex.out[i].nulls.cap >= (size_t)std::max<int64_t>(rows, 1) + 16));
    if (!fits) {
      size_t need = 0;
      for (auto& oc : ex.out) need += pitch((size_t)rows * oc.width + 16) + (oc.nullable ? pitch((size_t)rows + 16) : 0);
      for (auto& oc : ex.out) { oc.data.release(); oc.nulls.release(); }
      ex.out_arena.release();
      HIP_TRY(c, ex.out_arena.ensure(need));
      size_t off = 0;
      for (auto& oc : ex.out) { const size_t bytes = (size_t)rows * oc.width + 16; oc.data.set_view(ex.out_arena.as<char>() + off, bytes); off += pitch(bytes); }
      for (auto& oc : ex.out) if (oc.nullable) { oc.nulls.set_view(ex.out_arena.as<char>() + off, (size_t)rows + 16); off += pitch((size_t)rows + 16); }
    }
    ex.out_capacity = rows;
    return SSGPU_OK;
  }
  for (size_t i = 0; i < st.out_schema.size(); ++i) {
    OutCol& oc = ex.out[i];
    if (oc.data.view) oc.data.release();
    if (oc.nulls.view) oc.nulls.release();
    HIP_TRY(c, oc.data.ensure((size_t)std::max<int64_t>(rows, 1) * oc.width + 16));
    if (oc.nullable) HIP_TRY(c, oc.nulls.ensure((size_t)std::max<int64_t>(rows, 1) + 16));
  }
  ex.out_capacity = rows;
  return SSGPU_OK;
}

void fill_fast_slots(VmParams* P, const Stage& st) {
  for (size_t i = 0; i < st.aggs.size() && i < VM_FAST_SLOTS; ++i) {
    const int kind = st.aggs[i].slot == (int)i ? st.aggs[i].slot_kind : SLOT_COUNT;
    uint64_t i0 = 0, i1 = 0;
    const double pinf = __builtin_inf(), ninf = -__builtin_inf(), nzero = -0.0;
    switch (kind) {
      case SLOT_SUM_DD: memcpy(&i0, &nzero, 8); break;
      case SLOT_MIN_U64: i0 = ~0ull; break;
      case SLOT_MIN_F64: memcpy(&i0, &pinf, 8); break;
      case SLOT_MAX_F64: memcpy(&i0, &ninf, 8); break;
      case SLOT_FIRST: i1 = ~0ull; break;
      default: break;
    }
    P->slot_init0[i] = i0; P->slot_init1[i] = i1; P->slot_kind[i] = kind;
  }
}

int distinct_flags(ssgpu_ctx* c, const Stage& st, StageExec& ex, const InCols& in, ssgpu_column* out) {
  const uint32_t nk = (uint32_t)st.distinct_cols.size();
  if (nk > 16) { c->err = "DISTINCT aggregate under more than 15 group keys"; return SSGPU_ERROR_NOT_IMPLEMENTED; }
  const void* kdata[16] = {nullptr}; const uint8_t* knulls[16] = {nullptr}; uint32_t kwidth[16] = {0};
  for (uint32_t k = 0; k < nk; ++k) {
    const int col = st.distinct_cols[k];
    kdata[k] = in.cols[col].data; knulls[k] = in.cols[col].is_null; kwidth[k] = (uint32_t)dtype_width(st.in_schema[col].dtype);
  }
  HIP_TRY(c, ex.dflag.ensure((size_t)std::max<int64_t>(in.rows, 1)));
  HIP_TRY(c, ssgpu_launch_cluster_flags(kdata, knulls, kwidth, nk, (uint64_t)in.rows, ex.dflag.as<uint8_t>(), c->stream));
  out->data = ex.dflag.p; out->is_null = nullptr;
  return SSGPU_OK;
}

int prepare_scalar_emit(ssgpu_plan* p, size_t si, int* n_out);
int run_scalar_agg(ssgpu_plan* p, size_t si, const InCols& in0, int64_t row_id_base, bool stop_at_partial) {
  ssgpu_ctx* c = p->ctx; Stage& st = p->stages[si]; StageExec& ex = p->exec[si];
  InCols in = in0;
  if (!st.distinct_cols.empty()) {
    ssgpu_column f; const int rc = distinct_flags(c, st, ex, in0, &f); if (rc != SSGPU_OK) return rc;
    in.cols.push_back(f);
  }
  VmParams P;
  fill_params(&P, st.main, ex.lay, ex.prog_main, ex.n_instr_main, in, row_id_base);
  apply_joins(p, ex, st.main, &P);
  if (c->tile_map >= 2) P.flags |= VM_FLAG_XCD_CHUNKS;
  fill_fast_slots(&P, st);
  const int grid = grid_for(c, ex.lay, P.n_tiles);
  ex.grid = grid;
  const int ns = st.main.n_slots;
  HIP_TRY(c, ex.wg_partials.ensure((size_t)grid * ns * VM_WAVES * sizeof(VmAccRec)));
  HIP_TRY(c, ex.slot_recs.ensure((size_t)ns * sizeof(VmAccRec)));
  HIP_TRY(c, ex.state.ensure((size_t)ns * SSGPU_STATE_ARRAYS * sizeof(uint64_t)));
  if (!ex.slot_kind.p) {
    std::vector<int> kinds((size_t)ns, SLOT_COUNT);
    for (size_t i = 0; i < st.aggs.size(); ++i)
      if (st.aggs[i].slot == (int)i) kinds[i] = st.aggs[i].slot_kind;
    HIP_TRY(c, ex.slot_kind.ensure(kinds.size() * sizeof(int)));
    HIP_TRY(c, hipMemcpy(ex.slot_kind.p, kinds.data(), kinds.size() * sizeof(int), hipMemcpyHostToDevice));
  }
  P.wg_partials = ex.wg_partials.as<VmAccRec>();
  P.error_flag = ex.error_flag.as<unsigned int>();
  if (c->debug_timing) {
    HIP_TRY(c, ex.debug.ensure((size_t)grid * 4 * 8));
    P.debug = ex.debug.as<unsigned long long>();
  }
  { int rc = attach_pc_profile(c, ex, &P); if (rc != SSGPU_OK) return rc; }
  if (c->profile) HIP_TRY(c, hipEventRecord(p->ev_dom0, c->stream));
  HIP_TRY(c, launch_main(p, st, ex, P, ex.lay.K, grid));
  if (c->profile) HIP_TRY(c, hipEventRecord(p->ev_dom1, c->stream));
  { int rc = print_pc_profile(c, ex, st.main, P.n_instr); if (rc != SSGPU_OK) return rc; }
  int n_emit = 0;
  ex.emitted_with_finish = false;
  if (!stop_at_partial && c->fuse_emit) { const int rc = prepare_scalar_emit(p, si, &n_emit); if (rc != SSGPU_OK) return rc; ex.emitted_with_finish = true; }
  HIP_TRY(c, ssgpu_launch_finish_slots(ex.wg_partials.as<VmAccRec>(), ns, grid * VM_WAVES, ex.slot_kind.as<int>(),
                                       ex.slot_recs.as<VmAccRec>(), stop_at_partial ? ex.state.as<uint64_t>() : nullptr, c->stream,
                                       ex.emitted_with_finish ? ex.emit_descs.as<EmitDesc>() : nullptr, n_emit));
  p->counters.n_launches += 2;
  p->counters.tile_rows = P.tile_rows; p->counters.grid = grid; p->counters.lds_bytes = (int32_t)ex.lay.lds_bytes;
  if (c->debug_timing) {
    std::vector<unsigned long long> dbg((size_t)grid * 4);
    HIP_TRY(c, hipMemcpy(dbg.data(), ex.debug.p, dbg.size() * 8, hipMemcpyDeviceToHost));
    double tot = 0, wait = 0, tiles = 0;
    for (int g = 0; g < grid; ++g) { tot += (double)dbg[g * 4]; wait += (double)dbg[g * 4 + 1]; tiles += (double)dbg[g * 4 + 2]; }
    fprintf(stderr, "[ssgpu debug] grid=%d tiles/wg=%.1f cycles/wg=%.0f wait=%.1f%% cycles/tile=%.0f (wait %.0f)\n", grid, tiles / grid,
            tot / grid, 100.0 * wait / tot, tot / tiles, wait / tiles);
  }
  return SSGPU_OK;
}

static const int64_t kSeqSumPiece = 1 << 21;
static int run_seq_sums(ssgpu_plan* p, Stage& st, StageExec& ex, const InCols& in, const uint32_t* seg_id) {
  ssgpu_ctx* c = p->ctx;
  auto kind_of = [](int dtype) {
    switch (dtype) {
      case SSGPU_INT32: return 0; case SSGPU_UINT32: return 1; case SSGPU_INT64: return 2; case SSGPU_UINT64: return 3;
      case SSGPU_FLOAT: return 4; default: return 5;
    }
  };
  for (auto& q : st.seq_sums) {
    const void* src = in.cols[q.in_col].data;
    const uint8_t* src_nulls = st.in_schema[q.in_col].nullable ? in.cols[q.in_col].is_null : nullptr;
    uint8_t* dst_nulls = ex.out[q.out_col].nullable ? ex.out[q.out_col].nulls.as<uint8_t>() : nullptr;
    const int sk = kind_of(st.in_schema[q.in_col].dtype), dk = kind_of(st.out_schema[q.out_col].dtype);
    if (seg_id || in.rows <= kSeqSumPiece) {
      HIP_TRY(c, ssgpu_launch_seq_sum(src, src_nulls, sk, seg_id, (uint64_t)in.rows, ex.out[q.out_col].data.p, dst_nulls, dk, c->stream));
      p->counters.n_launches += 1;
      continue;
    }
    HIP_TRY(c, ex.total2.ensure(16));
    for (int64_t first = 0; first < in.rows; first += kSeqSumPiece) {
      const int64_t end = std::min<int64_t>(in.rows, first + kSeqSumPiece);
      HIP_TRY(c, ssgpu_launch_seq_sum(src, src_nulls, sk, nullptr, (uint64_t)end, ex.out[q.out_col].data.p, dst_nulls, dk, c->stream,
                                      (uint64_t)first, ex.total2.as<uint64_t>(), first > 0 ? 1 : 0));
      p->counters.n_launches += 1;
      if (end < in.rows) {
        HIP_TRY(c, hipStreamSynchronize(c->stream));
        if (p->interrupted.exchange(0)) { c->err = "interrupted"; return SSGPU_INTERRUPTED; }
      }
    }
  }
  return SSGPU_OK;
}

int prepare_scalar_emit(ssgpu_plan* p, size_t si, int* n_out) {
  ssgpu_ctx* c = p->ctx; Stage& st = p->stages[si]; StageExec& ex = p->exec[si];
  int rc = ensure_out_cols(c, st, ex, 1);
  if (rc != SSGPU_OK) return rc;
  *n_out = (int)st.aggs.size();
  if (!ex.emit_ready) {
    std::vector<EmitDesc> descs;
    for (size_t i = 0; i < st.aggs.size(); ++i) {
      EmitDesc d; d.data = ex.out[i].data.p; d.is_null = ex.out[i].nullable ? ex.out[i].nulls.as<uint8_t>() : nullptr;
      d.slot = st.aggs[i].slot; d.out_kind = st.aggs[i].emit_kind;
      descs.push_back(d);
    }
    HIP_TRY(c, ex.emit_descs.ensure(std::max<size_t>(descs.size(), 1) * sizeof(EmitDesc)));
    HIP_TRY(c, hipMemcpy(ex.emit_descs.p, descs.data(), descs.size() * sizeof(EmitDesc), hipMemcpyHostToDevice));
    ex.emit_ready = true;
  }
  return SSGPU_OK;
}

int emit_scalar_agg(ssgpu_plan* p, size_t si) {
  ssgpu_ctx* c = p->ctx; StageExec& ex = p->exec[si];
  int n_out = 0;
  const int rc = prepare_scalar_emit(p, si, &n_out);
  if (rc != SSGPU_OK) return rc;
  if (ex.emitted_with_finish) { ex.emitted_with_finish = false; ex.out_rows = 1; return SSGPU_OK; }
  HIP_TRY(c, ssgpu_launch_emit_scalar(ex.slot_recs.as<VmAccRec>(), ex.emit_descs.as<EmitDesc>(), n_out, c->stream));
  p->counters.n_launches += 1;
  ex.out_rows = 1;
  return SSGPU_OK;
}

int segment_ids(ssgpu_ctx* c, const Stage& st, StageExec& ex, const InCols& in, ssgpu_column* out) {
  const uint32_t nk = (uint32_t)st.segment_cols.size();
  if (nk > 16) { c->err = "AggregateClusters with more than 16 keys"; return SSGPU_ERROR_NOT_IMPLEMENTED; }
  const void* kdata[16] = {nullptr}; const uint8_t* knulls[16] = {nullptr}; uint32_t kwidth[16] = {0};
  void* okdata[16] = {nullptr}; uint8_t* oknulls[16] = {nullptr};
  for (uint32_t k = 0; k < nk; ++k) {
// ... 1180 lines not shown
                                        ex.out[q].width, idx, n_out, c->stream));
  }
  if (c->profile) HIP_TRY(c, hipEventRecord(p->ev_dom1, c->stream));
  p->counters.n_launches += 2 + (int)st.join_out.size();
  ex.out_rows = (int64_t)n_out;
  return SSGPU_OK;
}

int run_fold_tail(ssgpu_plan* p, size_t si, const InCols& in) {
  ssgpu_ctx* c = p->ctx; Stage& st = p->stages[si]; StageExec& ex = p->exec[si];
  if (st.fold_cut) {
    const int64_t keep = std::min<int64_t>(in.rows, p->be_capacity);
    int rc = ensure_out_cols(c, st, ex, keep);
    if (rc != SSGPU_OK) return rc;
    if (c->profile) HIP_TRY(c, hipEventRecord(p->ev_dom0, c->stream));
    for (size_t i = 0; i < st.out_schema.size() && keep > 0; ++i) {
      HIP_TRY(c, hipMemcpyAsync(ex.out[i].data.p, in.cols[i].data, (size_t)keep * ex.out[i].width, hipMemcpyDeviceToDevice, c->stream));
      if (ex.out[i].nullable) {
        if (st.in_schema[i].nullable && in.cols[i].is_null) HIP_TRY(c, hipMemcpyAsync(ex.out[i].nulls.p, in.cols[i].is_null, (size_t)keep, hipMemcpyDeviceToDevice, c->stream));
        else HIP_TRY(c, hipMemsetAsync(ex.out[i].nulls.p, 0, (size_t)keep, c->stream));
      }
    }
    if (c->profile) HIP_TRY(c, hipEventRecord(p->ev_dom1, c->stream));
    p->be_cut = -1;
    if (in.rows > keep) {
      unsigned long long next = 0;
      HIP_TRY(c, hipMemcpyAsync(&next, static_cast<const unsigned long long*>(in.cols[st.in_schema.size() - 1].data) + keep, 8, hipMemcpyDeviceToHost, c->stream));
      HIP_TRY(c, hipStreamSynchronize(c->stream));
      p->be_cut = (int64_t)next + p->be_base;
    }
    ex.out_rows = keep;
    return SSGPU_OK;
  }
  const int64_t keep = std::min<int64_t>(in.rows, st.fold_limit + 1);
  int rc = ensure_out_cols(c, st, ex, keep);
  if (rc != SSGPU_OK) return rc;
  auto kind_of = [](int dtype) {
    switch (dtype) {
      case SSGPU_INT32: case SSGPU_DATE: case SSGPU_STRING: return 0u; case SSGPU_UINT32: return 1u;
      case SSGPU_INT64: case SSGPU_DATETIME: return 2u; case SSGPU_UINT64: return 3u;
      case SSGPU_FLOAT: return 4u; case SSGPU_DOUBLE: return 5u; default: return 6u;
    }
  };
  std::vector<FoldTailColumn> cols(st.out_schema.size());
  for (size_t i = 0; i < cols.size(); ++i) {
    cols[i].src = in.cols[i].data; cols[i].src_nulls = st.in_schema[i].nullable ? in.cols[i].is_null : nullptr;
    cols[i].dst = ex.out[i].data.p; cols[i].dst_nulls = ex.out[i].nullable ? ex.out[i].nulls.as<uint8_t>() : nullptr;
    cols[i].op = (unsigned)st.fold_op[i]; cols[i].kind = kind_of(st.out_schema[i].dtype);
    const int by = i < st.fold_by.size() ? st.fold_by[i] : -1;
    cols[i].by = by >= 0 ? (const unsigned long long*)in.cols[by].data : nullptr;
    cols[i].by_nulls = by >= 0 && st.in_schema[by].nullable ? in.cols[by].is_null : nullptr;
  }
  HIP_TRY(c, ex.emit_descs.ensure(std::max<size_t>(cols.size(), 1) * sizeof(FoldTailColumn)));
  HIP_TRY(c, hipMemcpyAsync(ex.emit_descs.p, cols.data(), cols.size() * sizeof(FoldTailColumn), hipMemcpyHostToDevice, c->stream));
  HIP_TRY(c, hipStreamSynchronize(c->stream));
  if (c->profile) HIP_TRY(c, hipEventRecord(p->ev_dom0, c->stream));
  HIP_TRY(c, ssgpu_launch_fold_tail(ex.emit_descs.as<FoldTailColumn>(), (unsigned)cols.size(), (unsigned long long)in.rows, (unsigned long long)st.fold_limit, c->stream));
  if (c->profile) HIP_TRY(c, hipEventRecord(p->ev_dom1, c->stream));
  p->counters.n_launches += 1;
  ex.out_rows = keep;
  return SSGPU_OK;
}

static const void* rows_word(const StageExec& ex) { return ex.out_rows_dev ? ex.out_rows_dev : ex.total.p; }
int stage_rows(ssgpu_plan* p, size_t si, int64_t* rows) {
  ssgpu_ctx* c = p->ctx; StageExec& ex = p->exec[si];
  if (ex.out_rows < 0) {
    uint64_t total = 0;
    HIP_TRY(c, hipMemcpyAsync(&total, rows_word(ex), 8, hipMemcpyDeviceToHost, c->stream));
    HIP_TRY(c, hipStreamSynchronize(c->stream));
    ex.out_rows = (int64_t)total;
  }
  *rows = ex.out_rows;
  return SSGPU_OK;
}

int check_error_flags(ssgpu_plan* p);

int check_error_flags(ssgpu_plan* p) {
  ssgpu_ctx* c = p->ctx;
  std::vector<uint32_t> flags(p->exec.size(), 0);
  for (size_t i = 0; i < p->exec.size(); ++i)
    if (p->exec[i].error_flag.p)
      HIP_TRY(c, hipMemcpyAsync(&flags[i], p->exec[i].error_flag.p, 4, hipMemcpyDeviceToHost, c->stream));
  HIP_TRY(c, hipStreamSynchronize(c->stream));
  for (uint32_t& f : flags) {
    if (f & SSGPU_FLAG_NAN_IN_MINMAX) p->nan_seen = true;
    f &= 0xFFu;
  }
  for (uint32_t f : flags) {
    if (f == 3) { c->err = "decoupled look-back: a tile waited for an earlier tile's row count for too long and gave up"; return SSGPU_ERROR_HIP; }
    if (f == SSGPU_EVAL_ERROR_FOREIGN_KEY) {
      c->err = "No parent record with ID > " + std::to_string(std::max<int64_t>(p->aux_rows, 0));
      return SSGPU_ERROR_FOREIGN_KEY_INVALID;
    }
    if (f) {
      c->err = f == 2 ? "Evaluation error: invalid argument of a signaling math expression (negative input of SQRT)"
                      : "Evaluation error: division by zero in a signaling expression";
      return SSGPU_ERROR_EVALUATION_ERROR;
    }
  }
  return SSGPU_OK;
}

static int order_after_uploads(ssgpu_ctx* c) {
  if (!c->copy_pending.exchange(false, std::memory_order_acq_rel)) return SSGPU_OK;
  if (!c->copy_ev) HIP_TRY(c, hipEventCreateWithFlags(&c->copy_ev, hipEventDisableTiming));
  HIP_TRY(c, hipEventRecord(c->copy_ev, c->copy_stream));
  HIP_TRY(c, hipStreamWaitEvent(c->stream, c->copy_ev, 0));
  return SSGPU_OK;
}
int run_plan(ssgpu_plan* p, const ssgpu_column* cols, int32_t n_cols, int64_t rows, int64_t row_id_base, bool partial);

int settle_plan(ssgpu_plan* p) {
  if (!p->deferred) return SSGPU_OK;
  ssgpu_ctx* c = p->ctx;
  p->deferred = false;
  HIP_TRY(c, hipStreamSynchronize(c->stream));
  bool rerun = false;
  for (auto& ex : p->exec) {
    if (!ex.fb_pending) continue;
    const uint32_t* fb = static_cast<const uint32_t*>(ex.fb_host.p);
    const int kind = ex.fb_pending; ex.fb_pending = 0;
    if (fb[0] || (kind == 2 && (fb[1] || fb[3]))) { rerun = true; ex.steady = 0; }
    else if (kind == 1 && (uint64_t)fb[1] > 2ull * ex.steady_bypass + (uint64_t)(p->last_rows >> 6)) ex.steady = 0;
  }
  if (!rerun) return SSGPU_OK;
  std::vector<ssgpu_column> cols = p->last_cols;
  return run_plan(p, cols.data(), (int32_t)cols.size(), p->last_rows, p->last_base, p->last_partial);
}

int fix_nan_minmax(ssgpu_plan* p) {
  if (!p->nan_seen) return SSGPU_OK;
  p->nan_seen = false;
  if (p->desc.nan_exact || p->partial_pending) return SSGPU_OK;
  ssgpu_ctx* c = p->ctx;
  p->desc.nan_exact = true;
  std::vector<Stage> stages; Schema schema; std::string describe;
  Status s = lower_plan(p->desc, &stages, &schema, &describe);
  if (!s.ok()) { p->desc.nan_exact = false; return SSGPU_OK; }
  HIP_TRY(c, hipStreamSynchronize(c->stream));
  for (auto& ex : p->exec) { ex.rtc_main.drop(); ex.rtc_pscatter.drop(); ex.rtc_plain.drop(); ex.rtc_part.drop(); ex.rtc_resident.drop(); ex.rtc_hot.drop(); }
  for (auto& ex : p->exec) if (ex.fb_event) { (void)hipEventDestroy(ex.fb_event); ex.fb_event = nullptr; g_events.fetch_sub(1); }
  p->exec.clear();
  p->stages = stages; p->describe = describe;
  p->exec.resize(p->stages.size());
  std::vector<ssgpu_column> cols = p->last_cols;
  int rc = run_plan(p, cols.data(), (int32_t)cols.size(), p->last_rows, p->last_base, false);
  if (rc != SSGPU_OK) return rc;
  rc = settle_plan(p);
  if (rc != SSGPU_OK) return rc;
  rc = check_error_flags(p);
  p->nan_seen = false;
  return rc;
}

int run_plan(ssgpu_plan* p, const ssgpu_column* cols, int32_t n_cols, int64_t rows, int64_t row_id_base, bool partial) {
  ssgpu_ctx* c = p->ctx;
  if (!c || c->device < 0) { if (c) c->err = "no gfx950 device bound to this context (bind-only context)"; return SSGPU_ERROR_NO_DEVICE; }
  ssgpu_rtc_mode(!p->cached_only ? 0 : p->background && rows >= p->background_min_rows ? 2 : 1);
  p->run_row_end = row_id_base + rows;
  p->nan_seen = false;
  if (p->deferred) {
    p->deferred = false;
    for (auto& ex : p->exec) {
      if (!ex.fb_pending) continue;
      if (ex.fb_event) HIP_TRY(c, hipEventSynchronize(ex.fb_event)); else HIP_TRY(c, hipStreamSynchronize(c->stream));
      const uint32_t* fb = static_cast<const uint32_t*>(ex.fb_host.p);
      const int kind = ex.fb_pending; ex.fb_pending = 0;
      if (fb[0] || (kind == 2 && (fb[1] || fb[3]))) ex.steady = 0;
      else if (kind == 1 && (uint64_t)fb[1] > 2ull * ex.steady_bypass + (uint64_t)(p->last_rows >> 6)) ex.steady = 0;
    }
  }
  if (n_cols != (int)p->desc.input_schema.size()) { c->err = "column count does not match the plan's input schema"; return SSGPU_ERROR_ATTRIBUTE_COUNT_MISMATCH; }
  if (rows < 0) { c->err = "negative row count"; return SSGPU_ERROR_INVALID_ARGUMENT_VALUE; }
  if (p->interrupted.exchange(0)) { c->err = "interrupted"; return SSGPU_INTERRUPTED; }
  QuotaScope quota_scope(&p->quota);
  HIP_TRY(c, hipSetDevice(c->device));
  { const int orc = order_after_uploads(c); if (orc != SSGPU_OK) return orc; }
  memset(&p->counters, 0, sizeof(p->counters));
  { const int trc = ensure_dict_tables(p); if (trc != SSGPU_OK) return trc; }
  p->counters.rows_in = rows;
  p->result.fetched.assign(p->result.fetched.size(), false);
  for (ssgpu_dict*& cd : p->result.concat_dicts) { if (cd) ssgpu_dict_destroy(cd); cd = nullptr; }
  InCols in; in.cols.assign(cols, cols + n_cols); in.rows = rows;
  if (partial && !(p->stages.size() == 1 && p->stages[0].kind == STAGE_SCALAR_AGG)) {
    c->err = "partial runs need a plan whose only stage is a ScalarAggregate"; return SSGPU_ERROR_NOT_IMPLEMENTED;
  }
  for (size_t si = 0; si < p->stages.size(); ++si) {
    if (si == 0) ++p->n_runs;
    int rc = prepare_stage(p, si);
    if (rc != SSGPU_OK) return rc;
  }
  if (c->profile) {
    const int slot = (int)(p->profiled_runs % ssgpu_plan::kEventRing);
    if (!p->ring0[slot]) { HIP_TRY(c, hipEventCreate(&p->ring0[slot])); HIP_TRY(c, hipEventCreate(&p->ring1[slot])); g_events.fetch_add(2); }
    p->ev_dom0 = p->ring0[slot]; p->ev_dom1 = p->ring1[slot];
    ++p->profiled_runs;
    p->events_valid = false;
    if (c->profile_total) HIP_TRY(c, hipEventRecord(p->ev_begin, c->stream));
  }
  for (size_t si = 0; si < p->exec.size(); ++si)
    if (p->exec[si].error_flag.p && !p->keep_error_flags && !(si == 0 && p->stages[si].kind == STAGE_GROUP_AGG)) HIP_TRY(c, hipMemsetAsync(p->exec[si].error_flag.p, 0, sizeof(uint32_t), c->stream));
  int64_t alg_bytes = 0;
  for (size_t si = 0; si < p->stages.size(); ++si) {
    if (p->interrupted.exchange(0)) { c->err = "interrupted"; return SSGPU_INTERRUPTED; }
    Stage& st = p->stages[si];
    int rc = SSGPU_OK;
    alg_bytes += st.algorithmic_bytes_per_row * in.rows;
    rc = build_joins(p, st, p->exec[si]);
    if (rc != SSGPU_OK) return rc;
    switch (st.kind) {
      case STAGE_SCALAR_AGG:
        rc = run_scalar_agg(p, si, in, row_id_base, partial);
        if (rc == SSGPU_OK && !partial) rc = emit_scalar_agg(p, si);
        if (rc == SSGPU_OK && !partial && !st.seq_sums.empty()) rc = run_seq_sums(p, st, p->exec[si], in, nullptr);
        break;
      case STAGE_MATERIALIZE: rc = run_materialize(p, si, in, row_id_base); break;
      case STAGE_GROUP_AGG: rc = run_group_agg(p, si, in, row_id_base); break;
      case STAGE_SORT: rc = run_sort(p, si, in); break;
      case STAGE_CLUSTERS: rc = run_clusters(p, si, in, row_id_base); break;
      case STAGE_JOIN_EXPAND: rc = run_join_expand(p, si, in); break;
      case STAGE_FOLD_TAIL: rc = run_fold_tail(p, si, in); break;
      default: c->err = "stage kind not executable yet"; rc = SSGPU_ERROR_NOT_IMPLEMENTED; break;
    }
    if (rc != SSGPU_OK) return rc;
    if (si + 1 < p->stages.size()) {
      StageExec& ex = p->exec[si];
      const Stage& nx = p->stages[si + 1];
      const bool device_rows = c->async_handoff != 0 && !c->debug_timing && ex.out_rows < 0 && ex.out_capacity > 0 && nx.kind == STAGE_MATERIALIZE &&
                               !nx.has_filter && nx.distinct_cols.empty() && !nx.has_segment && !nx.has_rank && nx.joins.empty();
      int64_t r = 0;
      in.rows_dev = nullptr;
      if (device_rows) {
        r = ex.out_capacity;
        in.rows_dev = static_cast<const unsigned long long*>(rows_word(ex));
      } else {
        rc = stage_rows(p, si, &r);
        if (rc != SSGPU_OK) return rc;
        rc = check_error_flags(p);
        if (rc != SSGPU_OK) return rc;
      }
      in.cols.clear();
      for (auto& oc : ex.out) { ssgpu_column col; col.data = oc.data.p; col.is_null = oc.nullable ? oc.nulls.as<uint8_t>() : nullptr; in.cols.push_back(col); }
      in.rows = r;
      row_id_base = 0;
    }
  }
  if (c->profile && c->profile_total) { HIP_TRY(c, hipEventRecord(p->ev_end, c->stream)); p->events_valid = true; }
  p->counters.algorithmic_bytes = alg_bytes;
  p->last_rows = rows;
  p->last_cols.assign(cols, cols + n_cols); p->last_base = row_id_base; p->last_partial = partial;
  p->partial_pending = partial;
  return SSGPU_OK;
}

}

extern "C" {

int ssgpu_plan_run(ssgpu_plan* p, const ssgpu_column* cols, int32_t n_cols, int64_t rows, ssgpu_result** out) {
  if (!p) return SSGPU_ERROR_INVALID_ARGUMENT_VALUE;
  int rc = run_plan(p, cols, n_cols, rows, 0, false);
  if (rc != SSGPU_OK) return rc;
  if (!p->lazy_feedback) {
    rc = settle_plan(p);
    if (rc != SSGPU_OK) return rc;
    (void)check_error_flags(p);
    rc = fix_nan_minmax(p);
    if (rc != SSGPU_OK) return rc;
  }
  if (out) *out = &p->result;
  return SSGPU_OK;
}

int ssgpu_plan_run_best_effort(ssgpu_plan* p, const ssgpu_column* cols, int32_t n_cols, int64_t rows, int64_t start_row, int64_t* next_row, ssgpu_result** out) {
  if (!p || !next_row) return SSGPU_ERROR_INVALID_ARGUMENT_VALUE;
  ssgpu_ctx* c = p->ctx;
  if (!p->best_effort) { if (c) c->err = "ssgpu_plan_run_best_effort needs a plan whose root is a BestEffortGroupAggregate"; return SSGPU_ERROR_INVALID_ARGUMENT_VALUE; }
  if (n_cols != (int)p->desc.input_schema.size()) { c->err = "column count does not match the plan's input schema"; return SSGPU_ERROR_ATTRIBUTE_COUNT_MISMATCH; }
  if (start_row < 0 || start_row > rows) { c->err = "start_row outside the input"; return SSGPU_ERROR_INVALID_ARGUMENT_VALUE; }
  std::vector<ssgpu_column> win((size_t)n_cols);
  auto window = [&](int64_t s) {
    for (int i = 0; i < n_cols; ++i) {
      const size_t w = (size_t)dtype_width(p->desc.input_schema[i].dtype);
      win[i].data = cols[i].data ? static_cast<const char*>(cols[i].data) + (size_t)s * w : nullptr;
// ... 1177 lines not shown
  return SSGPU_OK;
}

int ssgpu_plan_counters(ssgpu_plan* p, ssgpu_counters* out) {
  if (!p || !out) return SSGPU_ERROR_INVALID_ARGUMENT_VALUE;
  ssgpu_ctx* c = p->ctx;
  if (c->device >= 0 && c->profile && p->profiled_runs > 0) {
    float ms = 0;
    if (p->events_valid) {
      HIP_TRY(c, hipEventSynchronize(p->ev_end));
      if (hipEventElapsedTime(&ms, p->ev_begin, p->ev_end) == hipSuccess) p->counters.kernel_ms = ms;
    } else if (p->ev_dom1) {
      HIP_TRY(c, hipStreamSynchronize(c->stream));
    }
    if (p->ev_dom0 && hipEventElapsedTime(&ms, p->ev_dom0, p->ev_dom1) == hipSuccess) p->counters.dominant_ms = ms;
  }
  *out = p->counters;
  return SSGPU_OK;
}

}

namespace {
struct ImageLayout {
  int64_t image_bytes = 0, unpacked_bytes = 0, valid_off = 0, trailer_off = 0;
  std::vector<int64_t> img_data, img_null, unp_data, unp_null;
  std::vector<uint32_t> width;
};
int64_t align16(int64_t v) { return (v + 15) & ~int64_t(15); }
bool image_layout(const Schema& schema, int64_t cap, int32_t n_images, ImageLayout* L) {
  if (cap < 0 || n_images < 1 || schema.size() * 2 > SSGPU_IMAGE_MAX_PIECES) return false;
  const size_t n = schema.size();
  L->img_data.assign(n, -1); L->img_null.assign(n, -1); L->unp_data.assign(n, -1); L->unp_null.assign(n, -1); L->width.assign(n, 0);
  int64_t io = SSGPU_IMAGE_HEADER, uo = 0;
  for (size_t i = 0; i < n; ++i) {
    const int w = dtype_width(schema[i].dtype);
    if (w == 0) return false;
    L->width[i] = (uint32_t)w;
    L->img_data[i] = io; io = align16(io + cap * w);
    L->unp_data[i] = uo; uo = align16(uo + (int64_t)n_images * cap * w);
    if (schema[i].nullable) {
      L->img_null[i] = io; io = align16(io + cap);
      L->unp_null[i] = uo; uo = align16(uo + (int64_t)n_images * cap);
    }
  }
  L->image_bytes = io;
  L->valid_off = uo; uo = align16(uo + (int64_t)n_images * cap);
  L->trailer_off = uo; uo += 32;
  L->unpacked_bytes = uo;
  return true;
}
}

extern "C" {

int ssgpu_plan_image_layout(const ssgpu_plan* p, int64_t capacity_rows, int32_t n_images, int64_t* image_bytes,
                            int64_t* unpacked_bytes, int64_t* offsets) {
  if (!p) return SSGPU_ERROR_INVALID_ARGUMENT_VALUE;
  ImageLayout L;
  if (!image_layout(p->result_schema, capacity_rows, n_images, &L)) {
    p->ctx->err = "result images need fixed-width columns, at most 46 of them, and a non-negative capacity";
    return SSGPU_ERROR_INVALID_ARGUMENT_VALUE;
  }
  if (image_bytes) *image_bytes = L.image_bytes;
  if (unpacked_bytes) *unpacked_bytes = L.unpacked_bytes;
  if (offsets) {
    const size_t n = p->result_schema.size();
    for (size_t i = 0; i < n; ++i) { offsets[4 * i] = L.img_data[i]; offsets[4 * i + 1] = L.img_null[i]; offsets[4 * i + 2] = L.unp_data[i]; offsets[4 * i + 3] = L.unp_null[i]; }
    offsets[4 * n] = -1; offsets[4 * n + 1] = -1; offsets[4 * n + 2] = L.valid_off; offsets[4 * n + 3] = -1;
  }
  return SSGPU_OK;
}

int ssgpu_result_pack_image(ssgpu_result* r, int64_t capacity_rows, void* image) {
  if (!r || !r->plan || r->plan->exec.empty() || !image) return SSGPU_ERROR_INVALID_ARGUMENT_VALUE;
  ssgpu_plan* p = r->plan; ssgpu_ctx* c = p->ctx;
  if (c->device < 0) return SSGPU_ERROR_NO_DEVICE;
  ImageLayout L;
  if (!image_layout(p->result_schema, capacity_rows, 1, &L)) { c->err = "result images need fixed-width columns and a non-negative capacity"; return SSGPU_ERROR_INVALID_ARGUMENT_VALUE; }
  StageExec& ex = p->exec.back();
  ImagePackParams P; memset(&P, 0, sizeof(P));
  P.image = image; P.capacity = (unsigned long long)capacity_rows;
  if (ex.out_rows >= 0) P.rows_host = (unsigned long long)ex.out_rows; else P.rows_dev = static_cast<const unsigned long long*>(rows_word(ex));
  for (auto& sx : p->exec) if (sx.error_flag.p && P.n_flags < 8) P.error_flags[P.n_flags++] = sx.error_flag.as<unsigned int>();
  for (auto& sx : p->exec) if (sx.fb_pending && sx.goverflow.p && P.n_retry + 2 <= 4) {
    P.retry_flags[P.n_retry++] = sx.goverflow.as<unsigned int>();
    if (sx.fb_pending == 2) P.retry_flags[P.n_retry++] = sx.goverflow.as<unsigned int>() + 1;
  }
  for (size_t i = 0; i < ex.out.size(); ++i) {
    ImagePiece& d = P.pieces[P.n_pieces++];
    d.src = ex.out[i].data.p; d.image_off = (unsigned long long)L.img_data[i]; d.width = L.width[i];
    if (L.img_null[i] >= 0) {
      ImagePiece& z = P.pieces[P.n_pieces++];
      z.src = ex.out[i].nullable ? ex.out[i].nulls.p : nullptr; z.image_off = (unsigned long long)L.img_null[i]; z.width = 1;
    }
  }
  HIP_TRY(c, ssgpu_launch_pack_image(P, c->stream));
  return SSGPU_OK;
}

int ssgpu_result_route_images(ssgpu_result* r, int32_t n_keys, int32_t n_dest, int64_t capacity_rows, void* images) {
  if (!r || !r->plan || r->plan->exec.empty() || !images || n_dest < 1 || n_dest > 256 || n_keys < 0 || n_keys > 16) return SSGPU_ERROR_INVALID_ARGUMENT_VALUE;
  ssgpu_plan* p = r->plan; ssgpu_ctx* c = p->ctx;
  if (c->device < 0) return SSGPU_ERROR_NO_DEVICE;
  if (n_keys > (int32_t)p->result_schema.size()) return SSGPU_ERROR_INVALID_ARGUMENT_VALUE;
  ImageLayout L;
  if (!image_layout(p->result_schema, capacity_rows, 1, &L)) { c->err = "result images need fixed-width columns and a non-negative capacity"; return SSGPU_ERROR_INVALID_ARGUMENT_VALUE; }
  StageExec& ex = p->exec.back();
  ImagePackParams P; memset(&P, 0, sizeof(P));
  ImageRoutePieces R; memset(&R, 0, sizeof(R));
  P.image = images; P.capacity = (unsigned long long)capacity_rows;
  const uint64_t rows_max = ex.out_rows >= 0 ? (uint64_t)ex.out_rows : (uint64_t)std::max<int64_t>(ex.out_capacity, 1);
  P.rows_host = rows_max;
  if (ex.out_rows < 0) P.rows_dev = static_cast<const unsigned long long*>(rows_word(ex));
  for (auto& sx : p->exec) if (sx.error_flag.p && P.n_flags < 8) P.error_flags[P.n_flags++] = sx.error_flag.as<unsigned int>();
  for (auto& sx : p->exec) if (sx.fb_pending && sx.goverflow.p && P.n_retry + 2 <= 4) {
    P.retry_flags[P.n_retry++] = sx.goverflow.as<unsigned int>();
    if (sx.fb_pending == 2) P.retry_flags[P.n_retry++] = sx.goverflow.as<unsigned int>() + 1;
  }
  for (size_t i = 0; i < ex.out.size(); ++i) {
    if ((int32_t)i < n_keys) { R.key_piece[i] = P.n_pieces; R.key_null_piece[i] = -1; }
    ImagePiece& d = P.pieces[P.n_pieces++];
    d.src = ex.out[i].data.p; d.image_off = (unsigned long long)L.img_data[i]; d.width = L.width[i];
    if (L.img_null[i] >= 0) {
      if ((int32_t)i < n_keys) R.key_null_piece[i] = (int)P.n_pieces;
      ImagePiece& z = P.pieces[P.n_pieces++];
      z.src = ex.out[i].nullable ? ex.out[i].nulls.p : nullptr; z.image_off = (unsigned long long)L.img_null[i]; z.width = 1;
    }
  }
  R.n_keys = (unsigned)n_keys; R.n_dest = (unsigned)n_dest; R.image_bytes = (unsigned long long)L.image_bytes;
  {
    const void* had = ex.route_scratch.p; const size_t had_cap = ex.route_scratch.cap;
    HIP_TRY(c, ex.route_scratch.ensure((256 + 2 * rows_max) * 4));
    if (ex.route_scratch.p != had || ex.route_scratch.cap != had_cap) HIP_TRY(c, hipMemsetAsync(ex.route_scratch.p, 0, 256 * 4, c->stream));
  }
  R.counters = ex.route_scratch.as<unsigned int>();
  HIP_TRY(c, ssgpu_launch_route_images(P, R, c->stream));
  return SSGPU_OK;
}

int ssgpu_images_unpack(ssgpu_plan* p, const void* images, int32_t n_images, int64_t capacity_rows, void* unpacked, ssgpu_column* cols) {
  if (!p || !images || !unpacked || !cols) return SSGPU_ERROR_INVALID_ARGUMENT_VALUE;
  ssgpu_ctx* c = p->ctx;
  if (c->device < 0) return SSGPU_ERROR_NO_DEVICE;
  ImageLayout L;
  if (!image_layout(p->result_schema, capacity_rows, n_images, &L)) { c->err = "result images need fixed-width columns and a non-negative capacity"; return SSGPU_ERROR_INVALID_ARGUMENT_VALUE; }
  ImageUnpackParams P; memset(&P, 0, sizeof(P));
  P.images = images; P.unpacked = unpacked; P.image_bytes = (unsigned long long)L.image_bytes; P.capacity = (unsigned long long)capacity_rows;
  P.valid_off = (unsigned long long)L.valid_off; P.trailer_off = (unsigned long long)L.trailer_off; P.n_images = (unsigned)n_images;
  char* base = static_cast<char*>(unpacked);
  const size_t n = p->result_schema.size();
  for (size_t i = 0; i < n; ++i) {
    ImagePiece& d = P.pieces[P.n_pieces++];
    d.image_off = (unsigned long long)L.img_data[i]; d.unpacked_off = (unsigned long long)L.unp_data[i]; d.width = L.width[i];
    cols[i].data = base + L.unp_data[i]; cols[i].is_null = nullptr;
    if (L.img_null[i] >= 0) {
      ImagePiece& z = P.pieces[P.n_pieces++];
      z.image_off = (unsigned long long)L.img_null[i]; z.unpacked_off = (unsigned long long)L.unp_null[i]; z.width = 1;
      cols[i].is_null = reinterpret_cast<const uint8_t*>(base + L.unp_null[i]);
    }
  }
  cols[n].data = base + L.valid_off; cols[n].is_null = nullptr;
  HIP_TRY(c, ssgpu_launch_unpack_images(P, c->stream));
  return SSGPU_OK;
}

}
```

### supersonic_amd/csrc/runtime_internal.h

```cpp
#ifndef SSGPU_RUNTIME_INTERNAL_H_
#define SSGPU_RUNTIME_INTERNAL_H_

#include <hip/hip_runtime_api.h>

#include <algorithm>
#include <atomic>
#include <map>
#include <mutex>
#include <stdio.h>
#include <stdlib.h>
#include <string>
#include <vector>

#include "engine.h"

using ssgpu::LowerOptions;
#define SSGPU_INTERNAL __attribute__((visibility("hidden")))

#define HIP_TRY(ctx, expr)                                                          \
  do {                                                                               \
    hipError_t _e = (expr);                                                          \
    if (_e != hipSuccess) {                                                          \
      (ctx)->err = _e == hipErrorOutOfMemory ? std::string("Memory exceeded: ") + #expr : std::string(#expr) + ": " + hipGetErrorString(_e); \
      return _e == hipErrorOutOfMemory ? SSGPU_ERROR_MEMORY_EXCEEDED : SSGPU_ERROR_HIP; \
    }                                                                                \
  } while (0)

struct ssgpu_ctx {
  std::atomic<int> refs{1};
  int device = -1;
  hipStream_t stream = nullptr, copy_stream = nullptr;
  std::atomic<bool> copy_pending{false};
  hipEvent_t copy_ev = nullptr;
  bool own_stream = false;
  int cu_count = 0;
  std::string err;
  LowerOptions opt;
  int64_t grid_limit = 0;
  int64_t out_arena = 1;
  int64_t tile_map = 1;
  int64_t wgs_per_cu = 3;
  int64_t group_capacity = 1 << 18;
  int64_t group_local = 1;
  int64_t group_partition = 1;
  int64_t part_n = 0;
  int64_t part_wgs_per_cu = 0;
  int64_t part_lds_target = 0;
  int64_t sort_records = 1;
  int64_t sort_hybrid = 1;
  int64_t group_slab = 1;
  int64_t group_scout = 1;
  int64_t group_scout_rows = 8 << 20;
  int64_t group_resident = 1;
  int64_t group_dense = 1;
  int64_t dense_parts = 0;
  int64_t dense_min_rows = 1 << 16;
  int64_t async_handoff = 1;
  int64_t lazy_feedback = 0;
  int64_t part_prefetch = 1;
  int64_t fuse_emit = 1;
  int64_t pscat_pipe = 1;
  int64_t pscat_threads = 0, pscat_rows = 0, pscat_wgs = 0;
  int64_t part_plain = 1;
  int64_t sort_compact = 1;
  int64_t sort_hi_digits = 4;
  int64_t part_agg_lds = 0;
  int64_t profile = 1;
  int64_t profile_total = 1;
  int64_t debug_timing = 0;
  int64_t specialize = 3;
  int64_t specialize_min_rows = 1 << 22;
};

struct MemQuota { int64_t limit = -1; int64_t used = 0; };
extern SSGPU_INTERNAL thread_local MemQuota* g_quota;
struct QuotaScope { MemQuota* saved; explicit QuotaScope(MemQuota* q) : saved(g_quota) { g_quota = q; } ~QuotaScope() { g_quota = saved; } };

extern SSGPU_INTERNAL std::atomic<long long> g_dev_bytes, g_pinned_bytes;

struct DevPool {
  std::mutex m;
  std::multimap<size_t, std::pair<void*, int>> blocks;
  size_t bytes = 0;
  size_t limit() { static const size_t v = [] { const char* e = getenv("SSGPU_POOL_MB"); return (size_t)(e ? atoll(e) : 4096) << 20; }(); return v; }
  bool park(void* p, size_t cap) {
    if (limit() == 0) return false;
    hipPointerAttribute_t attr;
    if (hipPointerGetAttributes(&attr, p) != hipSuccess) { (void)hipGetLastError(); return false; }
    const int dev = attr.device;
    std::lock_guard<std::mutex> lock(m);
    if (bytes + cap > limit() || blocks.size() >= 4096) return false;
    blocks.emplace(cap, std::make_pair(p, dev)); bytes += cap;
    return true;
  }
  void* take(size_t want, size_t* cap) {
    int dev = 0;
    if (limit() == 0 || hipGetDevice(&dev) != hipSuccess) return nullptr;
    const size_t most = want <= 4096 ? 4096 : want * 2;
    std::lock_guard<std::mutex> lock(m);
    for (auto it = blocks.lower_bound(want); it != blocks.end() && it->first <= most; ++it)
      if (it->second.second == dev) { void* p = it->second.first; *cap = it->first; bytes -= it->first; blocks.erase(it); return p; }
    return nullptr;
  }
  size_t trim(int dev);
  size_t parked(int dev) {
    std::lock_guard<std::mutex> lock(m);
    size_t n = 0;
    for (auto& b : blocks) if (dev < 0 || b.second.second == dev) n += b.first;
    return n;
  }
};
extern SSGPU_INTERNAL DevPool g_pool;
extern SSGPU_INTERNAL thread_local bool tls_park_released;

struct DevBuf {
  void* p = nullptr;
  size_t cap = 0;
  bool view = false;
  MemQuota* q = nullptr;
  ~DevBuf() { release(); }
  void release() {
    if (p && !view) {
      if (q) q->used -= (int64_t)cap;
      if (!(tls_park_released && g_pool.park(p, cap))) { (void)hipFree(p); g_dev_bytes.fetch_sub((long long)cap); }
    }
    p = nullptr; cap = 0; q = nullptr; view = false;
  }
  void set_view(void* ptr, size_t bytes) { release(); p = ptr; cap = bytes; view = true; }
  hipError_t ensure(size_t bytes) {
    if (bytes <= cap && p) return hipSuccess;
    if (view) return hipErrorInvalidValue;
    size_t want = std::max<size_t>(bytes, 256);
    MemQuota* Q = g_quota;
    if (Q && Q->limit >= 0 && Q->used - (q == Q ? (int64_t)cap : 0) + (int64_t)want > Q->limit) return hipErrorOutOfMemory;
    static const bool trace = getenv("SSGPU_TRACE") != nullptr;
    if (trace && want >= (64u << 20)) fprintf(stderr, "[ssgpu trace] device buffer %zu -> %zu MiB\n", cap >> 20, want >> 20);
    release();
    size_t pooled_cap = 0;
    if (void* pooled = (Q && Q->limit >= 0) ? nullptr : g_pool.take(want, &pooled_cap)) { p = pooled; cap = pooled_cap; q = Q; if (q) q->used += (int64_t)cap; return hipSuccess; }
    hipError_t e = hipMalloc(&p, want);
    if (e == hipErrorOutOfMemory) {
      (void)hipGetLastError();
      int dev = -1;
// ... 46 lines not shown
```

### supersonic_amd/csrc/vm.h

```cpp
#ifndef SSGPU_VM_H_
#define SSGPU_VM_H_

#ifdef __HIPCC_RTC__
typedef signed char int8_t; typedef unsigned char uint8_t; typedef short int16_t; typedef unsigned short uint16_t;
typedef int int32_t; typedef unsigned int uint32_t; typedef long int64_t; typedef unsigned long uint64_t; typedef unsigned long uintptr_t;
typedef int hipError_t; typedef struct ihipStream_t* hipStream_t;
#else
#include <stdint.h>
#endif

#define VM_NONE 0xFFFFFFFFu
enum { VM_MATH_EXP = 1, VM_MATH_LN, VM_MATH_LOG10, VM_MATH_LOG2, VM_MATH_SIN, VM_MATH_COS, VM_MATH_TAN, VM_MATH_ASIN, VM_MATH_ACOS,
       VM_MATH_ATAN, VM_MATH_SINH, VM_MATH_COSH, VM_MATH_TANH, VM_MATH_ASINH, VM_MATH_ACOSH, VM_MATH_ATANH, VM_MATH_POW, VM_MATH_ATAN2 };
#ifndef VM_THREADS
#define VM_THREADS 256
#endif
#ifndef VM_PF_UNITS
#define VM_PF_UNITS 8
#endif
#ifndef VM_WAVES_PER_EU
#define VM_WAVES_PER_EU 4
#endif
#ifndef VM_STAGE_PRIO
#define VM_STAGE_PRIO 1
// ... 113 lines not shown
  uint64_t imm;
};
static_assert(sizeof(VmInstr) == 32, "VmInstr must be 32 bytes");

struct VmStagedCol {
  const void* src;
  uint32_t lds_off;
  uint32_t width;
};

struct VmOutCol {
  void* dst;
  uint32_t width;
  uint32_t pad;
};

struct VmAccRec {
  uint64_t v0;
  uint64_t v1;
  uint64_t cnt;
  uint64_t pad;
};

struct VmGroupTable {
  unsigned long long* keys;
  unsigned long long* acc;
  unsigned int* cnt;
  unsigned int* overflow;
  uint32_t capacity_mask;
  uint32_t local_capacity;
  uint32_t local_sub;
  uint32_t local_sub_capacity;
  uint32_t local_keys_off;
  uint32_t local_acc_off;
  uint32_t local_cnt_off;
  uint32_t local_stride;
  uint32_t local_pad;
  uint32_t n_gaggs;
  const unsigned long long* acc_init;
  const unsigned int* merge_op;
  unsigned int* stats;
};
#define VM_MERGE_ADD_U64 0u
#define VM_MERGE_MIN_U64 1u
#define VM_MERGE_MAX_U64 2u
#define VM_MERGE_ADD_F64 3u
#define VM_MERGE_ADD_F64_HI 4u
#define VM_SLOT_LOCAL 0x80000000u
#define VM_KEY_EMPTY 0xFFFFFFFFFFFFFFFFull

struct VmJoin {
  const unsigned long long* keys;
  const unsigned int* rows;
  const unsigned int* special;
  uint32_t capacity_mask;
  uint32_t answer_slot;
  const unsigned long long* keys_hi;
};
struct VmJoinCol { const void* data; const unsigned char* is_null; };
#define VM_MAX_JOINS 2
#define VM_MAX_JOIN_COLS 24

struct VmParams {
  const VmInstr* prog;
  int32_t n_instr;
  int32_t n_staged;
  int32_t n_outputs;
  int32_t n_slots;
  int64_t n_rows;
  int64_t row_id_base;
  int32_t tile_rows;
  int32_t n_tiles;
  uint32_t acc_lds_off;
  uint32_t scratch_lds_off;
  uint32_t imm_pool_lds_off;
  uint32_t const_lds_off;
  uint32_t lds_bytes;
  int32_t count_sub_k;
  uint32_t flags;
  uint64_t slot_init0[VM_FAST_SLOTS];
  uint64_t slot_init1[VM_FAST_SLOTS];
  int32_t slot_kind[VM_FAST_SLOTS];
  VmAccRec* wg_partials;
  unsigned int* tile_counts;
  uint32_t part_n;
  uint32_t part_lds_off;
  uint32_t part_seg_cap;
  unsigned int* part_overflow;
  const unsigned int* tile_offsets;
  const unsigned long long* n_rows_dev;
  unsigned int* error_flag;
  unsigned long long* debug;
  unsigned long long* debug_pc;
  uint32_t debug_pc_lds_off;
  uint32_t uses_math;
  VmGroupTable group;
  VmJoin join[VM_MAX_JOINS];
  VmJoinCol join_cols[VM_MAX_JOIN_COLS];
  VmStagedCol staged[VM_MAX_STAGED];
  VmOutCol outputs[VM_MAX_OUTPUTS];
};
static_assert(sizeof(VmParams) <= 4096, "VmParams must fit the 4 KiB kernel-argument block");

#define VM_FLAG_XCD_CHUNKS 1u

#ifndef __HIPCC__
static inline const char* vm_op_name(uint16_t op) {
  static const char* names[] = {
#define X(n) #n,
      VM_OPS(X)
#undef X
  };
  return op < VM_OP_COUNT_ ? names[op] : "?";
}
#endif

#define SSGPU_EVAL_ERROR_FOREIGN_KEY 4u

#define SSGPU_FLAG_NAN_IN_MINMAX 0x100u

#endif
```

Before: 103.7 billion rows/s.

## Fuse scalar-aggregate finish into main kernel via last-block ticket, per-block partial folding

Each workgroup now folds its per-wave accumulators in LDS before writing a single partial per slot, laid out slot-major. An optional last-block-done path (atomic ticket counter) lets the final workgroup fold all partials, write slot records, state and emitted scalars, which removes the separate finish launch. Error flags are double-buffered so the next run's flag is cleared on device instead of by a memset. The initial tile prefetch is also hoisted ahead of LDS initialization. The fused path is off by default (scalar_fused_finish=0), so by default the changes are the smaller partial buffer, the wave-level finish kernel, the error-word handling and the earlier prefetch.

Result: no change. 103.9 billion rows/s, median of 2 (+0.1%).

```diff
diff --git a/supersonic_amd/csrc/launch.h b/supersonic_amd/csrc/launch.h
--- a/supersonic_amd/csrc/launch.h
+++ b/supersonic_amd/csrc/launch.h
@@ -206,7 +206,8 @@
 hipError_t ssgpu_pipeline_set_max_lds(int bytes);
 hipError_t ssgpu_launch_finish_slots(const VmAccRec* partials, int n_slots, int n_parts, const int* slot_kind,
                                      VmAccRec* out, uint64_t* state , hipStream_t stream,
-                                     const EmitDesc* descs = nullptr, int n_out = 0 );
+                                     const EmitDesc* descs = nullptr, int n_out = 0 ,
+                                     unsigned int* next_error_flag = nullptr );
 hipError_t ssgpu_launch_slots_to_state(const VmAccRec* recs, int n_slots, const int* slot_kind, uint64_t* state,
                                        hipStream_t stream);
 hipError_t ssgpu_launch_fold_state(const uint64_t* images, int n_images, uint64_t* state, int n_slots, const int* slot_kind, hipStream_t stream);
diff --git a/supersonic_amd/csrc/pipeline_kernels.hip b/supersonic_amd/csrc/pipeline_kernels.hip
--- a/supersonic_amd/csrc/pipeline_kernels.hip
+++ b/supersonic_amd/csrc/pipeline_kernels.hip
@@ -519,6 +519,139 @@
   }
 }
 
+__device__ __forceinline__ void combine_rec(int kind, VmAccRec& acc, const VmAccRec& r) {
+  if (r.cnt == 0) return;
+  switch (kind) {
+    case SLOT_COUNT:
+    case SLOT_SUM_INT: acc.v0 += r.v0; break;
+    case SLOT_SUM_DD: {
+      DD a; a.hi = u2d(acc.v0); a.lo = u2d(acc.v1);
+      DD b; b.hi = u2d(r.v0); b.lo = u2d(r.v1);
+      a = dd_add(a, b); acc.v0 = d2u(a.hi); acc.v1 = d2u(a.lo);
+    } break;
+    case SLOT_MIN_U64: acc.v0 = acc.cnt ? (r.v0 < acc.v0 ? r.v0 : acc.v0) : r.v0; break;
+    case SLOT_MAX_U64: acc.v0 = acc.cnt ? (r.v0 > acc.v0 ? r.v0 : acc.v0) : r.v0; break;
+    case SLOT_MIN_F64: acc.v0 = acc.cnt ? (u2d(r.v0) < u2d(acc.v0) ? r.v0 : acc.v0) : r.v0; break;
+    case SLOT_MAX_F64: acc.v0 = acc.cnt ? (u2d(acc.v0) < u2d(r.v0) ? r.v0 : acc.v0) : r.v0; break;
+    case SLOT_FIRST: if (!acc.cnt || r.v1 < acc.v1) { acc.v0 = r.v0; acc.v1 = r.v1; } break;
+    case SLOT_LAST: if (!acc.cnt || r.v1 >= acc.v1) { acc.v0 = r.v0; acc.v1 = r.v1; } break;
+  }
+  acc.cnt += r.cnt;
+}
+__device__ __forceinline__ VmAccRec rec_identity(int kind) {
+  VmAccRec r; r.v0 = 0; r.v1 = 0; r.cnt = 0; r.pad = 0;
+  if (kind == SLOT_SUM_DD) { r.v0 = d2u(-0.0); r.v1 = d2u(0.0); }
+  return r;
+}
+__device__ __forceinline__ void store_rec_write_through(VmAccRec* dst, const VmAccRec& r) {
+  typedef __attribute__((address_space(1))) u64 gu64;
+  gu64* const p = (gu64*)reinterpret_cast<u64*>(dst);
+  __hip_atomic_store(p + 0, r.v0, __ATOMIC_RELAXED, __HIP_MEMORY_SCOPE_AGENT);
+  __hip_atomic_store(p + 1, r.v1, __ATOMIC_RELAXED, __HIP_MEMORY_SCOPE_AGENT);
+  __hip_atomic_store(p + 2, r.cnt, __ATOMIC_RELAXED, __HIP_MEMORY_SCOPE_AGENT);
+  __hip_atomic_store(p + 3, 0ull, __ATOMIC_RELAXED, __HIP_MEMORY_SCOPE_AGENT);
+}
+__device__ __forceinline__ VmAccRec fold_recs_in_order(int kind, const VmAccRec* recs, int n) {
+  VmAccRec acc = rec_identity(kind);
+  for (int i = 0; i < n; ++i) { const VmAccRec r = recs[i]; combine_rec(kind, acc, r); }
+  return acc;
+}
+template <int CTRL> __device__ __forceinline__ VmAccRec rec_dpp(const VmAccRec& r) {
+  VmAccRec o; o.v0 = dpp64<CTRL>(r.v0); o.v1 = dpp64<CTRL>(r.v1); o.cnt = dpp64<CTRL>(r.cnt); o.pad = 0; return o;
+}
+__device__ __forceinline__ VmAccRec rec_readlane(const VmAccRec& r, int lane) {
+  VmAccRec o; o.v0 = readlane64(r.v0, lane); o.v1 = readlane64(r.v1, lane); o.cnt = readlane64(r.cnt, lane); o.pad = 0; return o;
+}
+__device__ __forceinline__ VmAccRec wave_tree_rec(int kind, VmAccRec v) {
+  VmAccRec o;
+  o = rec_dpp<DPP_QUAD_XOR1>(v); combine_rec(kind, v, o);
+  o = rec_dpp<DPP_QUAD_XOR2>(v); combine_rec(kind, v, o);
+  o = rec_dpp<DPP_ROW_ROR4>(v); combine_rec(kind, v, o);
+  o = rec_dpp<DPP_ROW_ROR8>(v); combine_rec(kind, v, o);
+  VmAccRec r0 = rec_readlane(v, 0), r2 = rec_readlane(v, 32);
+  const VmAccRec r1 = rec_readlane(v, 16), r3 = rec_readlane(v, 48);
+  combine_rec(kind, r0, r1); combine_rec(kind, r2, r3); combine_rec(kind, r0, r2);
+  return r0;
+}
+__device__ __forceinline__ VmAccRec fold_slot_wave(int kind, const VmAccRec* recs, int n, int t) {
+  VmAccRec v = rec_identity(kind);
+  for (int i0 = 0; i0 < n; i0 += VM_THREADS) {
+    VmAccRec r; r.v0 = 0; r.v1 = 0; r.cnt = 0; r.pad = 0;
+    if (i0 + t < n) r = recs[i0 + t];
+    combine_rec(kind, v, r);
+  }
+  return wave_tree_rec(kind, v);
+}
+#define VM_FOLD_BATCH 4
+__device__ __forceinline__ int slot_kind_at(const VmParams& P, int s) {
+  if (s >= VM_FAST_SLOTS) return P.slot_kinds[s];
+  int kind = 0;
+#pragma unroll
+  for (int j = 0; j < VM_FAST_SLOTS; ++j) kind = s == j ? P.slot_kind[j] : kind;
+  return kind;
+}
+__device__ __forceinline__ void fold_slots_wave(const int (&kind)[VM_FOLD_BATCH], const VmAccRec* recs, int s0, int n_slots, int n, int t,
+                                                VmAccRec (&out)[VM_FOLD_BATCH]) {
+#pragma unroll
+  for (int j = 0; j < VM_FOLD_BATCH; ++j) out[j] = rec_identity(kind[j]);
+  for (int i0 = 0; i0 < n; i0 += VM_THREADS) {
+    VmAccRec r[VM_FOLD_BATCH];
+#pragma unroll
+    for (int j = 0; j < VM_FOLD_BATCH; ++j) { r[j].v0 = 0; r[j].v1 = 0; r[j].cnt = 0; r[j].pad = 0; }
+    if (i0 + t < n) {
+#pragma unroll
+      for (int j = 0; j < VM_FOLD_BATCH; ++j) {
+        const int s = s0 + j < n_slots ? s0 + j : n_slots - 1;
+        const VmAccRec* const q = recs + (size_t)s * n + (i0 + t);
+        r[j].v0 = q->v0; r[j].v1 = q->v1; r[j].cnt = q->cnt;
+      }
+    }
+#pragma unroll
+    for (int j = 0; j < VM_FOLD_BATCH; ++j) combine_rec(kind[j], out[j], r[j]);
+  }
+#pragma unroll
+  for (int j = 0; j < VM_FOLD_BATCH; ++j) out[j] = wave_tree_rec(kind[j], out[j]);
+}
+__device__ __forceinline__ void slot_to_state(const VmAccRec r, int kind, int s, int n_slots, u64* __restrict__ state) {
+  u64* sum_i = state; u64* cnt = state + n_slots; u64* hi = state + 2 * n_slots; u64* lo = state + 3 * n_slots;
+  u64* mn = state + 4 * n_slots; u64* mx = state + 5 * n_slots;
+  u64* mnf = state + 6 * n_slots; u64* mxf = state + 7 * n_slots;
+  const bool fl = kind == SLOT_FIRST || kind == SLOT_LAST;
+  sum_i[s] = (kind == SLOT_SUM_INT || kind == SLOT_COUNT || fl) ? r.v0 : 0;
+  cnt[s] = r.cnt;
+  hi[s] = kind == SLOT_SUM_DD ? r.v0 : d2u(0.0);
+  lo[s] = kind == SLOT_SUM_DD ? r.v1 : d2u(0.0);
+  mn[s] = (kind == SLOT_MIN_U64 && r.cnt) ? (r.v0 ^ 0x8000000000000000ull) : (kind == SLOT_FIRST && r.cnt) ? (r.v1 ^ 0x8000000000000000ull) : 0x7FFFFFFFFFFFFFFFull;
+  mx[s] = (kind == SLOT_MAX_U64 && r.cnt) ? (r.v0 ^ 0x8000000000000000ull) : (kind == SLOT_LAST && r.cnt) ? (r.v1 ^ 0x8000000000000000ull) : 0x8000000000000000ull;
+  mnf[s] = (kind == SLOT_MIN_F64 && r.cnt) ? r.v0 : d2u(__builtin_inf());
+  mxf[s] = (kind == SLOT_MAX_F64 && r.cnt) ? r.v0 : d2u(-__builtin_inf());
+}
+__device__ __forceinline__ void emit_value(void* dst, size_t idx, int out_kind, u64 v0, u64 v1) {
+  switch (out_kind) {
+    case EMIT_U64: reinterpret_cast<u64*>(dst)[idx] = v0; break;
+    case EMIT_I64KEY: reinterpret_cast<i64*>(dst)[idx] = unkey_i64(v0); break;
+    case EMIT_U32: reinterpret_cast<u32*>(dst)[idx] = (u32)v0; break;
+    case EMIT_I32KEY: reinterpret_cast<i32*>(dst)[idx] = (i32)unkey_i64(v0); break;
+    case EMIT_F64: reinterpret_cast<double*>(dst)[idx] = u2d(v0); break;
+    case EMIT_F32: reinterpret_cast<float*>(dst)[idx] = (float)u2d(v0); break;
+    case EMIT_DD_F64: { double hi = u2d(v0), lo = u2d(v1);
+      reinterpret_cast<double*>(dst)[idx] = (lo == 0.0) ? hi : hi + lo; } break;
+    case EMIT_DDRES_F64: { const double hi = u2d(v0), lo = u2d(v1), sm = hi + lo, bp = sm - hi;
+      reinterpret_cast<double*>(dst)[idx] = (lo == 0.0) ? 0.0 : (hi - (sm - bp)) + (lo - bp); } break;
+    case EMIT_DD_F32: { double hi = u2d(v0), lo = u2d(v1);
+      reinterpret_cast<float*>(dst)[idx] = (float)((lo == 0.0) ? hi : hi + lo); } break;
+    case EMIT_U8: reinterpret_cast<u8*>(dst)[idx] = (u8)(v0 != 0); break;
+    default: break;
+  }
+}
+__device__ __forceinline__ void emit_scalar_one(const EmitDesc d, const VmAccRec r) {
+  if (d.out_kind == EMIT_CNT_U64 || d.out_kind == EMIT_CNT_U32)
+    emit_value(d.data, 0, d.out_kind == EMIT_CNT_U64 ? EMIT_U64 : EMIT_U32, r.cnt, 0);
+  else
+    emit_value(d.data, 0, d.out_kind, r.v0, r.v1);
+  if (d.is_null) d.is_null[0] = r.cnt == 0;
+}
+
 #ifndef SSGPU_RTC_PART
 template <int K, bool MATH>
 __global__ __launch_bounds__(VM_WG_THREADS, VM_WAVES_PER_EU) void ssgpu_pipeline_kernel(const VmParams P) {
@@ -540,6 +673,19 @@
   const int n_my_tiles = vm_n_tiles > vm_first_tile ? (vm_n_tiles - vm_first_tile + (int)gridDim.x - 1) / (int)gridDim.x : 0;
   const int n_units = STAGED_COUNT(P) * K;
 
+  u32x4 pf[VM_PF_UNITS];
+#pragma unroll
+  for (int u = 0; u < VM_PF_UNITS; ++u) pf[u] = u32x4{0u, 0u, 0u, 0u};
+  const int n_pf = n_units < VM_PF_UNITS ? n_units : VM_PF_UNITS;
+  {
+    const i64 tb = (i64)vm_first_tile * tile_rows;
+    if (n_my_tiles > 0 && tb + tile_rows <= vm_n_rows) {
+#pragma unroll
+      for (int u = 0; u < VM_PF_UNITS; ++u)
+        if (u < n_pf) load_unit<K>(P, u, tb, t, pf[u]);
+    }
+  }
+
   for (u32 o = (u32)t * 8u; o < (u32)P.n_slots * VM_ACC_STRIDE; o += VM_COMPUTE_THREADS * 8u)
     *reinterpret_cast<u64*>(smem + P.acc_lds_off + o) = 0ull;
   typedef u64 u64xS __attribute__((ext_vector_type(VM_FAST_SLOTS)));
@@ -583,19 +729,6 @@
   }
   PC_PROF(if (P.debug_pc) for (int i = t; i <= P.n_instr; i += VM_COMPUTE_THREADS) reinterpret_cast<u64*>(smem + P.debug_pc_lds_off)[i] = 0ull;)
   __syncthreads();
-
-  u32x4 pf[VM_PF_UNITS];
-#pragma unroll
-  for (int u = 0; u < VM_PF_UNITS; ++u) pf[u] = u32x4{0u, 0u, 0u, 0u};
-  const int n_pf = n_units < VM_PF_UNITS ? n_units : VM_PF_UNITS;
-  {
-    const i64 tb = (i64)vm_first_tile * tile_rows;
-    if (n_my_tiles > 0 && tb + tile_rows <= vm_n_rows) {
-#pragma unroll
-      for (int u = 0; u < VM_PF_UNITS; ++u)
-        if (u < n_pf) load_unit<K>(P, u, tb, t, pf[u]);
-    }
-  }
 
   u64 dbg_wait = 0;
   const u64 dbg_t0 = P.debug ? __builtin_amdgcn_s_memtime() : 0;
@@ -727,48 +860,59 @@
   }
 
   __syncthreads();
-  for (int s = t; s < P.n_slots; s += VM_COMPUTE_THREADS)
-    for (int w = 0; w < VM_WAVES; ++w)
-      P.wg_partials[((size_t)blockIdx.x * P.n_slots + s) * VM_WAVES + w] = *acc_rec(P, (u32)s, w);
+  const bool fin = P.fin_counter != nullptr;
+  for (int s = t; s < P.n_slots; s += VM_COMPUTE_THREADS) {
+    const VmAccRec r = fold_recs_in_order(slot_kind_at(P, s), acc_rec(P, (u32)s, 0), VM_WAVES);
+    VmAccRec* const dst = P.wg_partials + (size_t)s * gridDim.x + blockIdx.x;
+    if (fin) store_rec_write_through(dst, r); else *dst = r;
+  }
+  if (!fin) return;
+
+  asm volatile("s_waitcnt vmcnt(0)" ::: "memory");
+  __syncthreads();
+  u32* const fin_last = reinterpret_cast<u32*>(smem + P.scratch_lds_off);
+  if (t == 0) {
+    const u64 ticket = __hip_atomic_fetch_add(P.fin_counter, 1ull, __ATOMIC_RELAXED, __HIP_MEMORY_SCOPE_AGENT);
+    const bool last = ticket == P.fin_base + (u64)gridDim.x - 1ull;
+    *fin_last = last ? 1u : 0u;
+    if (last) {
+      __builtin_amdgcn_fence(__ATOMIC_ACQUIRE, "agent");
+      asm volatile("s_waitcnt vmcnt(0)" ::: "memory");
+    }
+  }
+  __syncthreads();
+  if (!*fin_last) return;
+  const int fin_grid = (int)gridDim.x;
+  const EmitDesc* const fin_descs = reinterpret_cast<const EmitDesc*>(P.fin_emit_descs);
+  EmitDesc fin_desc; fin_desc.data = nullptr; fin_desc.is_null = nullptr; fin_desc.slot = 0; fin_desc.out_kind = 0;
+  if (t < P.fin_n_emit) fin_desc = fin_descs[t];
+  for (int s0 = 0; s0 < P.n_slots; s0 += VM_FOLD_BATCH) {
+    int kind[VM_FOLD_BATCH];
+    VmAccRec part[VM_FOLD_BATCH];
+#pragma unroll
+    for (int j = 0; j < VM_FOLD_BATCH; ++j)
+      kind[j] = slot_kind_at(P, s0 + j < P.n_slots ? s0 + j : P.n_slots - 1);
+    fold_slots_wave(kind, P.wg_partials, s0, P.n_slots, fin_grid, t, part);
+#pragma unroll
+    for (int j = 0; j < VM_FOLD_BATCH; ++j)
+      if (lane == 0 && s0 + j < P.n_slots) *acc_rec(P, (u32)(s0 + j), wave) = part[j];
+  }
+  __syncthreads();
+  for (int s = t; s < P.n_slots; s += VM_COMPUTE_THREADS) {
+    const int kind = slot_kind_at(P, s);
+    const VmAccRec r = fold_recs_in_order(kind, acc_rec(P, (u32)s, 0), VM_WAVES);
+    P.fin_slot_recs[s] = r;
+    if (P.fin_state) slot_to_state(r, kind, s, P.n_slots, P.fin_state);
+    *acc_rec(P, (u32)s, 0) = r;
+  }
+  __syncthreads();
+  if (t < P.fin_n_emit) emit_scalar_one(fin_desc, *acc_rec(P, (u32)fin_desc.slot, 0));
+  for (int i = t + VM_COMPUTE_THREADS; i < P.fin_n_emit; i += VM_COMPUTE_THREADS) { const EmitDesc d = fin_descs[i]; emit_scalar_one(d, *acc_rec(P, (u32)d.slot, 0)); }
+  if (t == 0 && P.fin_next_error_flag) *P.fin_next_error_flag = 0u;
 }
 #endif
 
 #ifndef __HIPCC_RTC__
-
-__device__ __forceinline__ void combine_rec(int kind, VmAccRec& acc, const VmAccRec& r) {
-  if (r.cnt == 0) return;
-  switch (kind) {
-    case SLOT_COUNT:
-    case SLOT_SUM_INT: acc.v0 += r.v0; break;
-    case SLOT_SUM_DD: {
-      DD a; a.hi = u2d(acc.v0); a.lo = u2d(acc.v1);
-      DD b; b.hi = u2d(r.v0); b.lo = u2d(r.v1);
-      a = dd_add(a, b); acc.v0 = d2u(a.hi); acc.v1 = d2u(a.lo);
-    } break;
-    case SLOT_MIN_U64: acc.v0 = acc.cnt ? (r.v0 < acc.v0 ? r.v0 : acc.v0) : r.v0; break;
-    case SLOT_MAX_U64: acc.v0 = acc.cnt ? (r.v0 > acc.v0 ? r.v0 : acc.v0) : r.v0; break;
-    case SLOT_MIN_F64: acc.v0 = acc.cnt ? (u2d(r.v0) < u2d(acc.v0) ? r.v0 : acc.v0) : r.v0; break;
-    case SLOT_MAX_F64: acc.v0 = acc.cnt ? (u2d(acc.v0) < u2d(r.v0) ? r.v0 : acc.v0) : r.v0; break;
-    case SLOT_FIRST: if (!acc.cnt || r.v1 < acc.v1) { acc.v0 = r.v0; acc.v1 = r.v1; } break;
-    case SLOT_LAST: if (!acc.cnt || r.v1 >= acc.v1) { acc.v0 = r.v0; acc.v1 = r.v1; } break;
-  }
-  acc.cnt += r.cnt;
-}
-
-__device__ __forceinline__ void slot_to_state(const VmAccRec r, int kind, int s, int n_slots, u64* __restrict__ state) {
-  u64* sum_i = state; u64* cnt = state + n_slots; u64* hi = state + 2 * n_slots; u64* lo = state + 3 * n_slots;
-  u64* mn = state + 4 * n_slots; u64* mx = state + 5 * n_slots;
-  u64* mnf = state + 6 * n_slots; u64* mxf = state + 7 * n_slots;
-  const bool fl = kind == SLOT_FIRST || kind == SLOT_LAST;
-  sum_i[s] = (kind == SLOT_SUM_INT || kind == SLOT_COUNT || fl) ? r.v0 : 0;
-  cnt[s] = r.cnt;
-  hi[s] = kind == SLOT_SUM_DD ? r.v0 : d2u(0.0);
-  lo[s] = kind == SLOT_SUM_DD ? r.v1 : d2u(0.0);
-  mn[s] = (kind == SLOT_MIN_U64 && r.cnt) ? (r.v0 ^ 0x8000000000000000ull) : (kind == SLOT_FIRST && r.cnt) ? (r.v1 ^ 0x8000000000000000ull) : 0x7FFFFFFFFFFFFFFFull;
-  mx[s] = (kind == SLOT_MAX_U64 && r.cnt) ? (r.v0 ^ 0x8000000000000000ull) : (kind == SLOT_LAST && r.cnt) ? (r.v1 ^ 0x8000000000000000ull) : 0x8000000000000000ull;
-  mnf[s] = (kind == SLOT_MIN_F64 && r.cnt) ? r.v0 : d2u(__builtin_inf());
-  mxf[s] = (kind == SLOT_MAX_F64 && r.cnt) ? r.v0 : d2u(-__builtin_inf());
-}
 __device__ __forceinline__ VmAccRec state_to_slot(const u64* __restrict__ state, int kind, int s, int n_slots) {
   VmAccRec r; r.v0 = 0; r.v1 = 0; r.pad = 0;
   r.cnt = state[n_slots + s];
@@ -790,29 +934,26 @@
   return r;
 }
 
-__device__ __forceinline__ void emit_scalar_one(const EmitDesc d, const VmAccRec r);
-__global__ __launch_bounds__(256) void ssgpu_finish_slots_kernel(const VmAccRec* __restrict__ partials, int n_slots,
+__global__ __launch_bounds__(256) void ssgpu_finish_slots_kernel(const VmAccRec* partials, int n_slots,
                                                                  int n_parts, const int* __restrict__ slot_kind,
                                                                  VmAccRec* __restrict__ out, u64* __restrict__ state,
-                                                                 const EmitDesc* __restrict__ descs, int n_out) {
-  __shared__ VmAccRec tree[256];
+                                                                 const EmitDesc* __restrict__ descs, int n_out,
+                                                                 u32* __restrict__ next_error_flag) {
+  __shared__ VmAccRec waves[VM_WAVES + 1];
   const int s = blockIdx.x, t = threadIdx.x;
   const int kind = slot_kind[s];
-  VmAccRec acc; acc.v0 = 0; acc.v1 = 0; acc.cnt = 0; acc.pad = 0;
-  if (kind == SLOT_SUM_DD) { acc.v0 = d2u(-0.0); acc.v1 = d2u(0.0); }
-  for (int i = t; i < n_parts; i += 256) {
-    const VmAccRec r = partials[((size_t)(i / VM_WAVES) * n_slots + s) * VM_WAVES + (i % VM_WAVES)];
-    combine_rec(kind, acc, r);
-  }
-  tree[t] = acc;
+  const VmAccRec w = fold_slot_wave(kind, partials + (size_t)s * n_parts, n_parts, t);
+  if ((t & 63) == 0) waves[t >> 6] = w;
   __syncthreads();
-  for (int stride = 128; stride > 0; stride >>= 1) {
-    if (t < stride) { VmAccRec a = tree[t]; combine_rec(kind, a, tree[t + stride]); tree[t] = a; }
-    __syncthreads();
-  }
-  if (t == 0) { out[s] = tree[0]; if (state) slot_to_state(tree[0], kind, s, n_slots, state); }
+  if (t == 0) {
+    const VmAccRec r = fold_recs_in_order(kind, waves, VM_WAVES);
+    out[s] = r; if (state) slot_to_state(r, kind, s, n_slots, state);
+    waves[VM_WAVES] = r;
+  }
+  __syncthreads();
   if (descs)
-    for (int i = t; i < n_out; i += 256) { const EmitDesc d = descs[i]; if (d.slot == s) emit_scalar_one(d, tree[0]); }
+    for (int i = t; i < n_out; i += 256) { const EmitDesc d = descs[i]; if (d.slot == s) emit_scalar_one(d, waves[VM_WAVES]); }
+  if (next_error_flag && s == 0 && t == 0) *next_error_flag = 0u;
 }
 
 __global__ void ssgpu_slots_to_state_kernel(const VmAccRec* __restrict__ recs, int n_slots,
@@ -828,34 +969,6 @@
   recs[s] = state_to_slot(state, slot_kind[s], s, n_slots);
 }
 
-
-__device__ __forceinline__ void emit_value(void* dst, size_t idx, int out_kind, u64 v0, u64 v1) {
-  switch (out_kind) {
-    case EMIT_U64: reinterpret_cast<u64*>(dst)[idx] = v0; break;
-    case EMIT_I64KEY: reinterpret_cast<i64*>(dst)[idx] = unkey_i64(v0); break;
-    case EMIT_U32: reinterpret_cast<u32*>(dst)[idx] = (u32)v0; break;
-    case EMIT_I32KEY: reinterpret_cast<i32*>(dst)[idx] = (i32)unkey_i64(v0); break;
-    case EMIT_F64: reinterpret_cast<double*>(dst)[idx] = u2d(v0); break;
-    case EMIT_F32: reinterpret_cast<float*>(dst)[idx] = (float)u2d(v0); break;
-    case EMIT_DD_F64: { double hi = u2d(v0), lo = u2d(v1);
-      reinterpret_cast<double*>(dst)[idx] = (lo == 0.0) ? hi : hi + lo; } break;
-    case EMIT_DDRES_F64: { const double hi = u2d(v0), lo = u2d(v1), sm = hi + lo, bp = sm - hi;
-      reinterpret_cast<double*>(dst)[idx] = (lo == 0.0) ? 0.0 : (hi - (sm - bp)) + (lo - bp); } break;
-    case EMIT_DD_F32: { double hi = u2d(v0), lo = u2d(v1);
-      reinterpret_cast<float*>(dst)[idx] = (float)((lo == 0.0) ? hi : hi + lo); } break;
-    case EMIT_U8: reinterpret_cast<u8*>(dst)[idx] = (u8)(v0 != 0); break;
-    default: break;
-  }
-}
-
-
-__device__ __forceinline__ void emit_scalar_one(const EmitDesc d, const VmAccRec r) {
-  if (d.out_kind == EMIT_CNT_U64 || d.out_kind == EMIT_CNT_U32)
-    emit_value(d.data, 0, d.out_kind == EMIT_CNT_U64 ? EMIT_U64 : EMIT_U32, r.cnt, 0);
-  else
-    emit_value(d.data, 0, d.out_kind, r.v0, r.v1);
-  if (d.is_null) d.is_null[0] = r.cnt == 0;
-}
 __global__ void ssgpu_emit_scalar_kernel(const VmAccRec* __restrict__ recs, const EmitDesc* __restrict__ descs,
                                          int n_out) {
   int i = blockIdx.x * blockDim.x + threadIdx.x;
@@ -1807,8 +1920,8 @@
   return e;
 }
 hipError_t ssgpu_launch_finish_slots(const VmAccRec* partials, int n_slots, int n_parts, const int* slot_kind,
-                                     VmAccRec* out, uint64_t* state, hipStream_t stream, const EmitDesc* descs, int n_out) {
-  hipLaunchKernelGGL(ssgpu_finish_slots_kernel, dim3(n_slots), dim3(256), 0, stream, partials, n_slots, n_parts, slot_kind, out, (u64*)state, descs, n_out);
+                                     VmAccRec* out, uint64_t* state, hipStream_t stream, const EmitDesc* descs, int n_out, unsigned int* next_error_flag) {
+  hipLaunchKernelGGL(ssgpu_finish_slots_kernel, dim3(n_slots), dim3(256), 0, stream, partials, n_slots, n_parts, slot_kind, out, (u64*)state, descs, n_out, next_error_flag);
   return hipGetLastError();
 }
 hipError_t ssgpu_launch_slots_to_state(const VmAccRec* recs, int n_slots, const int* slot_kind, uint64_t* state, hipStream_t stream) {
diff --git a/supersonic_amd/csrc/runtime.cpp b/supersonic_amd/csrc/runtime.cpp
--- a/supersonic_amd/csrc/runtime.cpp
+++ b/supersonic_amd/csrc/runtime.cpp
@@ -119,6 +119,11 @@
   std::vector<VmJoin> vm_joins;
   uint32_t capacity = 0;
   DevBuf error_flag;
+  int err_word = 1;
+  bool err_dirty[2] = {false, false};
+  unsigned int* error_word() const { return error_flag.as<unsigned int>() + err_word; }
+  DevBuf fin_counter;
+  uint64_t fin_base = 0;
   DevBuf debug, debug_pc, total2;
   DevBuf skeys_a, skeys_b, skeys_c, sidx_a, sidx_b, shist, soffs, seg_id, sstatus, sticket, srecs, dflag;
   DevBuf rank_first, rank_of_seg, rank_row, rank_own;
@@ -336,6 +341,7 @@
   else if (k == "pscat_wgs") c->pscat_wgs = value;
   else if (k == "pscat_pipe") c->pscat_pipe = value;
   else if (k == "fuse_emit") c->fuse_emit = value;
+  else if (k == "scalar_fused_finish") c->scalar_fused_finish = value;
   else if (k == "part_prefetch") c->part_prefetch = value;
   else if (k == "lazy_feedback") c->lazy_feedback = value;
   else if (k == "async_handoff") c->async_handoff = value;
@@ -869,7 +875,11 @@
     rc = upload_program(c, st.count_pass, ex.lay_count, &ex.prog_count, &ex.n_instr_count, &p->host_prog_scratch);
     if (rc != SSGPU_OK) return rc;
   }
-  HIP_TRY(c, ex.error_flag.ensure(sizeof(uint32_t)));
+  if (!ex.error_flag.p) {
+    HIP_TRY(c, ex.error_flag.ensure(2 * sizeof(uint32_t)));
+    HIP_TRY(c, hipMemsetAsync(ex.error_flag.p, 0, 2 * sizeof(uint32_t), c->stream));
+    if (st.kind != STAGE_SCALAR_AGG) ex.err_word = 0;
+  }
   return SSGPU_OK;
 }
 
@@ -1161,6 +1171,15 @@
 }
 
 int prepare_scalar_emit(ssgpu_plan* p, size_t si, int* n_out);
+static bool scalar_fused(const ssgpu_ctx* c) { return c->scalar_fused_finish != 0 && !c->debug_timing; }
+static int error_word_begin(ssgpu_plan* p, StageExec& ex) {
+  ssgpu_ctx* c = p->ctx;
+  if (p->keep_error_flags) return SSGPU_OK;
+  ex.err_word ^= 1;
+  if (ex.err_dirty[ex.err_word] || c->debug_timing) HIP_TRY(c, hipMemsetAsync(ex.error_word(), 0, sizeof(uint32_t), c->stream));
+  ex.err_dirty[ex.err_word] = true;
+  return SSGPU_OK;
+}
 int run_scalar_agg(ssgpu_plan* p, size_t si, const InCols& in0, int64_t row_id_base, bool stop_at_partial) {
   ssgpu_ctx* c = p->ctx; Stage& st = p->stages[si]; StageExec& ex = p->exec[si];
   InCols in = in0;
@@ -1176,7 +1195,7 @@
   const int grid = grid_for(c, ex.lay, P.n_tiles);
   ex.grid = grid;
   const int ns = st.main.n_slots;
-  HIP_TRY(c, ex.wg_partials.ensure((size_t)grid * ns * VM_WAVES * sizeof(VmAccRec)));
+  HIP_TRY(c, ex.wg_partials.ensure((size_t)grid * ns * sizeof(VmAccRec)));
   HIP_TRY(c, ex.slot_recs.ensure((size_t)ns * sizeof(VmAccRec)));
   HIP_TRY(c, ex.state.ensure((size_t)ns * SSGPU_STATE_ARRAYS * sizeof(uint64_t)));
   if (!ex.slot_kind.p) {
@@ -1187,23 +1206,47 @@
     HIP_TRY(c, hipMemcpy(ex.slot_kind.p, kinds.data(), kinds.size() * sizeof(int), hipMemcpyHostToDevice));
   }
   P.wg_partials = ex.wg_partials.as<VmAccRec>();
-  P.error_flag = ex.error_flag.as<unsigned int>();
+  P.slot_kinds = ex.slot_kind.as<int32_t>();
+  P.error_flag = ex.error_word();
   if (c->debug_timing) {
     HIP_TRY(c, ex.debug.ensure((size_t)grid * 4 * 8));
     P.debug = ex.debug.as<unsigned long long>();
   }
   { int rc = attach_pc_profile(c, ex, &P); if (rc != SSGPU_OK) return rc; }
+  int n_emit = 0;
+  ex.emitted_with_finish = false;
+  if (!stop_at_partial && c->fuse_emit) { const int rc = prepare_scalar_emit(p, si, &n_emit); if (rc != SSGPU_OK) return rc; ex.emitted_with_finish = true; }
+  const bool fused = scalar_fused(c);
+  if (fused) {
+    if (!ex.fin_counter.p) {
+      HIP_TRY(c, ex.fin_counter.ensure(sizeof(uint64_t)));
+      HIP_TRY(c, hipMemsetAsync(ex.fin_counter.p, 0, sizeof(uint64_t), c->stream));
+      ex.fin_base = 0;
+    }
+    P.fin_counter = ex.fin_counter.as<unsigned long long>();
+    P.fin_base = ex.fin_base;
+    P.fin_slot_recs = ex.slot_recs.as<VmAccRec>();
+    P.fin_state = stop_at_partial ? ex.state.as<unsigned long long>() : nullptr;
+    P.fin_emit_descs = ex.emitted_with_finish ? ex.emit_descs.p : nullptr;
+    P.fin_n_emit = n_emit;
+    P.fin_next_error_flag = p->keep_error_flags ? nullptr : ex.error_flag.as<unsigned int>() + (ex.err_word ^ 1);
+  }
   if (c->profile) HIP_TRY(c, hipEventRecord(p->ev_dom0, c->stream));
   HIP_TRY(c, launch_main(p, st, ex, P, ex.lay.K, grid));
   if (c->profile) HIP_TRY(c, hipEventRecord(p->ev_dom1, c->stream));
-  { int rc = print_pc_profile(c, ex, st.main, P.n_instr); if (rc != SSGPU_OK) return rc; }
-  int n_emit = 0;
-  ex.emitted_with_finish = false;
-  if (!stop_at_partial && c->fuse_emit) { const int rc = prepare_scalar_emit(p, si, &n_emit); if (rc != SSGPU_OK) return rc; ex.emitted_with_finish = true; }
-  HIP_TRY(c, ssgpu_launch_finish_slots(ex.wg_partials.as<VmAccRec>(), ns, grid * VM_WAVES, ex.slot_kind.as<int>(),
-                                       ex.slot_recs.as<VmAccRec>(), stop_at_partial ? ex.state.as<uint64_t>() : nullptr, c->stream,
-                                       ex.emitted_with_finish ? ex.emit_descs.as<EmitDesc>() : nullptr, n_emit));
-  p->counters.n_launches += 2;
+  if (fused) {
+    ex.fin_base += (uint64_t)grid;
+    if (!p->keep_error_flags) ex.err_dirty[ex.err_word ^ 1] = false;
+    p->counters.n_launches += 1;
+  } else {
+    { int rc = print_pc_profile(c, ex, st.main, P.n_instr); if (rc != SSGPU_OK) return rc; }
+    unsigned int* const next_word = (p->keep_error_flags || c->debug_timing) ? nullptr : ex.error_flag.as<unsigned int>() + (ex.err_word ^ 1);
+    HIP_TRY(c, ssgpu_launch_finish_slots(ex.wg_partials.as<VmAccRec>(), ns, grid, ex.slot_kind.as<int>(),
+                                         ex.slot_recs.as<VmAccRec>(), stop_at_partial ? ex.state.as<uint64_t>() : nullptr, c->stream,
+                                         ex.emitted_with_finish ? ex.emit_descs.as<EmitDesc>() : nullptr, n_emit, next_word));
+    if (next_word) ex.err_dirty[ex.err_word ^ 1] = false;
+    p->counters.n_launches += 2;
+  }
   p->counters.tile_rows = P.tile_rows; p->counters.grid = grid; p->counters.lds_bytes = (int32_t)ex.lay.lds_bytes;
   if (c->debug_timing) {
     std::vector<unsigned long long> dbg((size_t)grid * 4);
@@ -2550,7 +2593,7 @@
   std::vector<uint32_t> flags(p->exec.size(), 0);
   for (size_t i = 0; i < p->exec.size(); ++i)
     if (p->exec[i].error_flag.p)
-      HIP_TRY(c, hipMemcpyAsync(&flags[i], p->exec[i].error_flag.p, 4, hipMemcpyDeviceToHost, c->stream));
+      HIP_TRY(c, hipMemcpyAsync(&flags[i], p->exec[i].error_word(), 4, hipMemcpyDeviceToHost, c->stream));
   HIP_TRY(c, hipStreamSynchronize(c->stream));
   for (uint32_t& f : flags) {
     if (f & SSGPU_FLAG_NAN_IN_MINMAX) p->nan_seen = true;
@@ -2668,8 +2711,11 @@
     p->events_valid = false;
     if (c->profile_total) HIP_TRY(c, hipEventRecord(p->ev_begin, c->stream));
   }
-  for (size_t si = 0; si < p->exec.size(); ++si)
-    if (p->exec[si].error_flag.p && !p->keep_error_flags && !(si == 0 && p->stages[si].kind == STAGE_GROUP_AGG)) HIP_TRY(c, hipMemsetAsync(p->exec[si].error_flag.p, 0, sizeof(uint32_t), c->stream));
+  for (size_t si = 0; si < p->exec.size(); ++si) {
+    if (!p->exec[si].error_flag.p) continue;
+    if (p->stages[si].kind == STAGE_SCALAR_AGG) { const int erc = error_word_begin(p, p->exec[si]); if (erc != SSGPU_OK) return erc; continue; }
+    if (!p->keep_error_flags && !(si == 0 && p->stages[si].kind == STAGE_GROUP_AGG)) HIP_TRY(c, hipMemsetAsync(p->exec[si].error_flag.p, 0, sizeof(uint32_t), c->stream));
+  }
   int64_t alg_bytes = 0;
   for (size_t si = 0; si < p->stages.size(); ++si) {
     if (p->interrupted.exchange(0)) { c->err = "interrupted"; return SSGPU_INTERRUPTED; }
@@ -4013,7 +4059,7 @@
   ImagePackParams P; memset(&P, 0, sizeof(P));
   P.image = image; P.capacity = (unsigned long long)capacity_rows;
   if (ex.out_rows >= 0) P.rows_host = (unsigned long long)ex.out_rows; else P.rows_dev = static_cast<const unsigned long long*>(rows_word(ex));
-  for (auto& sx : p->exec) if (sx.error_flag.p && P.n_flags < 8) P.error_flags[P.n_flags++] = sx.error_flag.as<unsigned int>();
+  for (auto& sx : p->exec) if (sx.error_flag.p && P.n_flags < 8) P.error_flags[P.n_flags++] = sx.error_word();
   for (auto& sx : p->exec) if (sx.fb_pending && sx.goverflow.p && P.n_retry + 2 <= 4) {
     P.retry_flags[P.n_retry++] = sx.goverflow.as<unsigned int>();
     if (sx.fb_pending == 2) P.retry_flags[P.n_retry++] = sx.goverflow.as<unsigned int>() + 1;
@@ -4044,7 +4090,7 @@
   const uint64_t rows_max = ex.out_rows >= 0 ? (uint64_t)ex.out_rows : (uint64_t)std::max<int64_t>(ex.out_capacity, 1);
   P.rows_host = rows_max;
   if (ex.out_rows < 0) P.rows_dev = static_cast<const unsigned long long*>(rows_word(ex));
-  for (auto& sx : p->exec) if (sx.error_flag.p && P.n_flags < 8) P.error_flags[P.n_flags++] = sx.error_flag.as<unsigned int>();
+  for (auto& sx : p->exec) if (sx.error_flag.p && P.n_flags < 8) P.error_flags[P.n_flags++] = sx.error_word();
   for (auto& sx : p->exec) if (sx.fb_pending && sx.goverflow.p && P.n_retry + 2 <= 4) {
     P.retry_flags[P.n_retry++] = sx.goverflow.as<unsigned int>();
     if (sx.fb_pending == 2) P.retry_flags[P.n_retry++] = sx.goverflow.as<unsigned int>() + 1;
diff --git a/supersonic_amd/csrc/runtime_internal.h b/supersonic_amd/csrc/runtime_internal.h
--- a/supersonic_amd/csrc/runtime_internal.h
+++ b/supersonic_amd/csrc/runtime_internal.h
@@ -59,6 +59,7 @@
   int64_t lazy_feedback = 0;
   int64_t part_prefetch = 1;
   int64_t fuse_emit = 1;
+  int64_t scalar_fused_finish = 0;
   int64_t pscat_pipe = 1;
   int64_t pscat_threads = 0, pscat_rows = 0, pscat_wgs = 0;
   int64_t part_plain = 1;
diff --git a/supersonic_amd/csrc/vm.h b/supersonic_amd/csrc/vm.h
--- a/supersonic_amd/csrc/vm.h
+++ b/supersonic_amd/csrc/vm.h
@@ -219,6 +219,15 @@
   uint64_t slot_init1[VM_FAST_SLOTS];
   int32_t slot_kind[VM_FAST_SLOTS];
   VmAccRec* wg_partials;
+  const int32_t* slot_kinds;
+  unsigned long long* fin_counter;
+  unsigned long long fin_base;
+  VmAccRec* fin_slot_recs;
+  unsigned long long* fin_state;
+  const void* fin_emit_descs;
+  int32_t fin_n_emit;
+  int32_t fin_pad;
+  unsigned int* fin_next_error_flag;
   unsigned int* tile_counts;
   uint32_t part_n;
   uint32_t part_lds_off;
```
